# weifengliu-ssslab/Benchmark_SpMV_using_CSR5

Measured on AMD Instinct MI355X. Metric: fp64 SpMV GFLOPS, higher is better.
Workload: dtype f64

## Files before the change

### benchmark_spmv_using_csr5_amd/csrc/csr5_internal.h

```cpp
#pragma once

#include <hip/hip_runtime.h>
#include <stdint.h>

#include "csr5hip.h"

namespace csr5 {

constexpr int OMEGA = CSR5HIP_OMEGA;
#ifndef CSR5_WAVES_PER_BLOCK
#define CSR5_WAVES_PER_BLOCK 1
#endif
constexpr int WAVES_PER_BLOCK = CSR5_WAVES_PER_BLOCK;
constexpr int BLOCK = OMEGA * WAVES_PER_BLOCK;
constexpr int FMT_WAVES_PER_BLOCK = 2;
constexpr int FMT_BLOCK = OMEGA * FMT_WAVES_PER_BLOCK;
constexpr int BIT_SS = 6;
constexpr uint32_t ROW_MASK = 0x7FFFFFFFu;
constexpr int STAMP_WORD = 8;
constexpr int COUNTER_WORDS = 16;
constexpr int NUM_XCD = 8;
constexpr int RUN_SERIAL_MAX = 64;
#ifndef CSR5_XWIN_BYTES
#define CSR5_XWIN_BYTES 4096
#endif
constexpr int XWIN_BYTES = CSR5_XWIN_BYTES;
constexpr int xwin_elems(int value_size) { return XWIN_BYTES / value_size; }
constexpr int XWIN_MIN_COVER_PCT = 30;

constexpr int bit_y_of(int sigma)
{
    int base = 2, b = 1;
    while (base < OMEGA * sigma) { base *= 2; b++; }
    return b;
}
constexpr int num_packet_of(int sigma) { return (bit_y_of(sigma) + BIT_SS + sigma + 31) / 32; }

struct Geometry {
    int m, n, nnz;
    int sigma;
    int bit_y, bit_all, num_packet;
    int p;
    int tile_elems;
    int tail_start;
    int defer;
};

struct DeviceArrays {
    const int32_t *row_ptr;
    int32_t *col;
    void *val;
    uint32_t *tile_ptr;
    uint32_t *tile_desc;
    int32_t *offset_ptr;
    int32_t *offset;
    void *calibrator;
    void *carry_acc;
    uint32_t *carry_cnt;
    uint32_t *carry_meta;
    uint32_t *tile_hdr;
    uint32_t *counters;
    const int32_t *hot_cols;
    const int32_t *hot_count;
    const int32_t *hot_tile0;
    int hot_slabs, hot_capacity;
    void *range_lead;
    uint32_t *range_head;
    const uint16_t *col_lo;
    const uint8_t *col_hi;
    const int32_t *slab_off;
    int slab_shift, slab_bits;
    const void *xperm;
    const int32_t *cold_base;
    const int32_t *cold_cols;
    int cold_total;
    const float *val32;
    const uint32_t *col16;
    const int32_t *base16;
    const uint32_t *col31;
};

hipError_t launch_row_scan(const Geometry &g, const DeviceArrays &d, hipStream_t s);
hipError_t launch_tile_desc(const Geometry &g, const DeviceArrays &d, hipStream_t s);
size_t offset_scan_tmp_bytes(int entries);
hipError_t launch_offset_scan(const Geometry &g, const DeviceArrays &d, void *tmp, size_t tmp_bytes, hipStream_t s);
hipError_t launch_desc_offset(const Geometry &g, const DeviceArrays &d, hipStream_t s);
hipError_t launch_transpose(const Geometry &g, const DeviceArrays &d, int value_type, bool r2c,
                            hipStream_t s);
hipError_t launch_transpose_values(const Geometry &g, const DeviceArrays &d, int value_type, hipStream_t s);
hipError_t launch_tile_tables(const Geometry &g, const DeviceArrays &d, int value_size, uint32_t *host_words, bool export_only,
                              hipStream_t s);
hipError_t launch_col16(const Geometry &g, const DeviceArrays &d, uint32_t *col16, int32_t *base16, uint32_t *wide_tiles,
                        hipStream_t s);
constexpr int COL16_SPAN = 32768;
constexpr bool col16_sigma(int sigma) { return sigma == 8 || sigma == 12 || sigma == 16 || sigma == 24 || sigma == 32; }
hipError_t launch_col31(const Geometry &g, const DeviceArrays &d, uint32_t *col31, hipStream_t s);
constexpr bool col31_sigma(int sigma) { return sigma >= 4 && sigma <= 8; }
hipError_t launch_warmup(hipStream_t s);
hipError_t launch_validate_csr(int m, int n, int nnz, const int32_t *row_ptr, const int32_t *col, uint32_t *flag,
                               hipStream_t s);

hipError_t slab_scan_tmp_bytes(size_t items, size_t *bytes);
hipError_t slab_select_tmp_bytes(int nnz, size_t *bytes);
hipError_t slab_partition(const Geometry &g, const DeviceArrays &d, int value_type, int S, int bits, int shift,
                          uint32_t *hist, void *scan_tmp, size_t scan_tmp_bytes, int32_t *col2, void *val2,
                          uint32_t *key2, hipStream_t s);
hipError_t slab_count_segments(int nnz, const uint32_t *key2, void *tmp, unsigned int *d_count, hipStream_t s);
hipError_t slab_segments(int nnz, const uint32_t *key2, const void *tmp, int32_t *row_ptr2, unsigned char *rowidx, hipStream_t s);
size_t slab_base_words(int m, int S);
hipError_t slab_tables(int m, int m2, int nnz, int S, int p, const int32_t *row_ptr, int32_t *row_ptr2, const uint32_t *key2,
                       const uint32_t *chunk_start, uint32_t *base, uint32_t *nonempty, hipStream_t s);
hipError_t slab_hot_select(int n, int nnz, int S, int bits, int shift, int capacity, int min_count, int sample_stride,
                           const int32_t *col, uint32_t *cnt, void *hotmap, uint32_t *chist, uint32_t *thr,
                           int32_t *hot_cols, int32_t *hot_count, unsigned long long *covered, hipStream_t s);
hipError_t slab_hot_finish(int S, int p_hist, int p, int T, int nnz, int capacity, const uint32_t *chunk_start,
                           int32_t *hot_count, int32_t *tile0, int32_t *slab_off, hipStream_t s);
size_t slab_cold_words(int n, int S, int bits, int shift);
hipError_t slab_cold_sort_tmp_bytes(size_t total, int slab_bits, size_t *bytes);
hipError_t slab_hot_pack(int n, int nnz, int T, int p, int S, int bits, int shift, const int32_t *slab_off, const void *hotmap,
                         const uint32_t *cnt, const uint32_t *key2, int32_t *col2, uint16_t *col_lo, uint8_t *col_hi, uint8_t *ref, uint32_t *rank_of,
                         uint32_t *keys, uint32_t *keys_sorted, uint32_t *src_sorted, void *sort_tmp, size_t sort_tmp_bytes,
                         int32_t *cold_base, int32_t *cold_cols, hipStream_t s);
size_t slab_local_columns(int n, int bits, int shift);
size_t slab_hotmap_bytes(int n, int S, int bits, int shift);
int slab_hot_buckets();
hipError_t launch_slab_combine(int m, int tail_start, int zero_empty, int S, int value_type, const uint32_t *base,
                               const unsigned char *rowidx, const uint32_t *nonempty, const void *P, int segments, void *y,
                               hipStream_t s);

hipError_t launch_refresh_values(const Geometry &g, const uint32_t *tile_ptr, int value_type, bool pieces, const uint32_t *src,
                                 const void *in, void *out, hipStream_t s);
hipError_t refresh_map_tmp_bytes(int nnz, int bits, size_t *bytes);
hipError_t refresh_build_map(const Geometry &g, const DeviceArrays &d, int bits, int shift, void *tmp, size_t tmp_bytes,
                             uint32_t *src, hipStream_t s);

hipError_t companion_tmp_bytes(int n, int nnz, size_t *bytes);
hipError_t companion_build(const Geometry &g, const DeviceArrays &d, int value_size, void *tmp, size_t tmp_bytes,
                           int32_t *row_ptr_t, int32_t *col_t, void *val_t, uint32_t *map, hipStream_t s);
hipError_t companion_gather(int nnz, int value_size, const uint32_t *map, const void *in, void *out, hipStream_t s);

struct SpmvOptions {
    int mode;
    int xcd_remap;
    int x_window;
    int lds_y;
    int stream_nt;
    int long_runs;
    int hot;
    int col16;
    int col31;
};
constexpr int DEFER_AUTO_LONG_ROW = 128;
constexpr int DEFER_AUTO_MIN_TILES_LONG = 3000;
constexpr int DEFER_AUTO_MIN_TILE_SIGMA = 500000;
constexpr int HOT_AUTO_MIN_COVER_PCT = 25;
constexpr long long HOT_AUTO_MIN_COVERED_BEYOND = 5000000;
constexpr int HOT_LDS_BYTES = 128 * 1024;
constexpr int HOT_WAVE_LDS = 4096;
#ifndef CSR5_HOT_WAVES
#define CSR5_HOT_WAVES 8
#endif
constexpr int HOT_WAVES = CSR5_HOT_WAVES;
constexpr int HOT_WGS_PER_XCD = 32;
constexpr int HOT_RANGES_PER_SLAB = HOT_WGS_PER_XCD * HOT_WAVES;
#ifndef CSR5_HOT_DEPTH
#define CSR5_HOT_DEPTH 2
#endif
struct HotParams {
    int slabs, rounds, capacity;
    const int32_t *count;
    const int32_t *tile0;
    const uint16_t *col_lo;
    const uint8_t *col_hi;
    const int32_t *slab_off;
    const void *xp;
    const int32_t *cold_base;
    int cold_total;
};
constexpr int hot_child_sigma(int value_size) { return HOT_WAVE_LDS / (OMEGA * value_size); }
hipError_t launch_spmv(const Geometry &g, const DeviceArrays &d, int value_type, const void *x,
                       void *y, const SpmvOptions &opt, hipStream_t s);
hipError_t launch_spmm(const Geometry &g, const DeviceArrays &d, int value_type, const void *X, int ldx, int k, void *Y, int ldy,
                       void *work, int zero_empty, int xcd_remap, hipStream_t s);
constexpr int spmm_block_width(int k) { return k <= 1 ? 1 : k <= 2 ? 2 : k <= 4 ? 4 : 8; }
hipError_t launch_sddmm(const Geometry &g, const DeviceArrays &d, int value_type, const void *U, int ldu, const void *V, int ldv, int k,
                        void *out, hipStream_t s);
hipError_t launch_row_softmax(int m, const int32_t *row_ptr, int value_type, const void *scores, void *out, hipStream_t s);
hipError_t launch_row_softmax_grad(int m, const int32_t *row_ptr, int value_type, const void *p, const void *g, void *out,
                                   hipStream_t s);
struct AttCall {
    int heads, groups, k, d;
    const void *Q;
    int ldq;
    const void *K;
    int ldk;
    const void *V;
    int ldv;
    void *O;
    int ldo;
    double scale;
    const void *slopes;
    const void *B;
    int ldb;
    const void *a;
    double negative_slope;
};
struct AttBwdCall : AttCall {
    const void *dO;
    int lddo;
    void *dQ;
    int lddq;
    void *dK;
    int lddk;
    void *dV;
    int lddv;
    void *work;
    void *dS;
    int ldds;
    void *dAr;
    int lddar;
    const Geometry *gt;
    const DeviceArrays *dt;
    const uint32_t *map;
};
enum AttVariant { ATT_PLAIN, ATT_BIASED, ATT_EDGE, ATT_GAT };
using AttLaunch = hipError_t(const Geometry &, const DeviceArrays &, const AttCall &, hipStream_t);
using AttBwdLaunch = hipError_t(const Geometry &, const DeviceArrays &, const AttBwdCall &, hipStream_t);
hipError_t launch_mha(const Geometry &g, const DeviceArrays &d, int value_type, const AttCall &c, hipStream_t s);
hipError_t launch_mha_biased(const Geometry &g, const DeviceArrays &d, int value_type, const AttCall &c, hipStream_t s);
hipError_t launch_mha_edge(const Geometry &g, const DeviceArrays &d, int value_type, const AttCall &c, hipStream_t s);
hipError_t launch_gat(const Geometry &g, const DeviceArrays &d, int value_type, const AttCall &c, hipStream_t s);
hipError_t launch_mha_lowp(const Geometry &g, const DeviceArrays &d, int operand_type, const AttCall &c, hipStream_t s);
hipError_t launch_mha_bwd(const Geometry &g, const DeviceArrays &d, int value_type, const AttBwdCall &c, hipStream_t s);
hipError_t launch_mha_biased_bwd(const Geometry &g, const DeviceArrays &d, int value_type, const AttBwdCall &c, hipStream_t s);
hipError_t launch_mha_edge_bwd(const Geometry &g, const DeviceArrays &d, int value_type, const AttBwdCall &c, hipStream_t s);
hipError_t launch_gat_bwd(const Geometry &g, const DeviceArrays &d, int value_type, const AttBwdCall &c, hipStream_t s);
hipError_t launch_mha_lowp_bwd(const Geometry &g, const DeviceArrays &d, int operand_type, const AttBwdCall &c, hipStream_t s);
hipError_t launch_spmv_hot(const Geometry &g, const DeviceArrays &d, int value_type, const void *x, void *y,
                           const SpmvOptions &opt, hipStream_t s);
hipError_t prepare_spmv_hot(const Geometry &g, const DeviceArrays &d, int value_type, const SpmvOptions &opt);
hipError_t launch_fp32_exact(const double *v, size_t n, unsigned *flag, hipStream_t s);
hipError_t launch_narrow(const double *v, size_t n, float *o, int tile_elems, int transposed_tiles, hipStream_t s);
hipError_t launch_range_heads(const Geometry &g, const DeviceArrays &d, hipStream_t s);
hipError_t launch_x_permute(const Geometry &g, const DeviceArrays &d, int value_type, const void *x, hipStream_t s);

}
```

### benchmark_spmv_using_csr5_amd/csrc/csr5_slab.hip

```cpp
#include "csr5_internal.h"
#include "csr5_slabmap.h"

#include <rocprim/device/device_radix_sort.hpp>
#include <rocprim/device/device_scan.hpp>
#include <rocprim/iterator/counting_iterator.hpp>

namespace csr5 {

constexpr int SLAB_BLOCK = 256;
constexpr int SLAB_MAX = 64;
constexpr uint32_t SLAB_KEY_FIRST = 0x80000000u;

__host__ __device__ inline size_t slab_hot_groups(int n, int shift, int bits) { return (slab_local_count(n, shift, bits) + 127) / 128; }
__device__ __forceinline__ bool hot_lookup(const uint4 w, uint32_t bit, uint32_t &below)
{
    const unsigned long long lo = (unsigned long long)w.x | ((unsigned long long)w.y << 32);
    const unsigned long long hi = (unsigned long long)w.z | ((unsigned long long)w.w << 32);
    const unsigned long long word = bit < 64 ? lo : hi;
    const uint32_t b = bit & 63;
    below = (uint32_t)__popcll(word & ((1ull << b) - 1ull)) + (bit < 64 ? 0u : (uint32_t)__popcll(lo));
    return (word >> b) & 1ull;
}

__device__ __forceinline__ int upper_bound_i32(const int32_t *__restrict__ a, int key, int size)
{
    int lo = 0, hi = size;
    while (lo < hi) {
        const int mid = (int)(((unsigned)lo + (unsigned)hi) >> 1);
        if (a[mid] <= key)
            lo = mid + 1;
        else
            hi = mid;
    }
    return lo;
}

__device__ __forceinline__ bool tile_is_transposed(const Geometry &g, const uint32_t *tile_ptr, int t)
{
    return t < g.p - 1 && tile_ptr[t] != tile_ptr[t + 1];
}

constexpr int HIST_TILES = 16, HIST_PAD = OMEGA + 1;
__global__ void __launch_bounds__(SLAB_BLOCK)
k_slab_hist(Geometry g, const int32_t *__restrict__ col, int S, int bits, int shift, uint32_t *__restrict__ hist)
{
    extern __shared__ uint32_t hist_lds[];
    __shared__ uint32_t sh[SLAB_MAX][HIST_TILES];
    const int lane = threadIdx.x & (OMEGA - 1), wave = threadIdx.x >> 6;
    uint32_t *mine = hist_lds + (size_t)wave * S * HIST_PAD;
    const int t0 = blockIdx.x * HIST_TILES;
    for (int i = wave; i < HIST_TILES; i += SLAB_BLOCK / OMEGA) {
        const int t = t0 + i;
        uint32_t total = 0;
        if (t < g.p) {
            for (int k = 0; k < S; k++)
                mine[k * HIST_PAD + lane] = 0;
            const size_t base = (size_t)t * g.tile_elems;
            const int E = (int)((size_t)g.nnz - base < (size_t)g.tile_elems ? (size_t)g.nnz - base : (size_t)g.tile_elems);
            constexpr int AHEAD = 8;
            for (int q0 = 0; q0 < E; q0 += AHEAD * OMEGA) {
                int32_t c[AHEAD];
#pragma unroll
                for (int u = 0; u < AHEAD; u++) {
                    const int q = q0 + u * OMEGA + lane;
                    c[u] = col[base + (q < E ? q : E - 1)];
                }
#pragma unroll
                for (int u = 0; u < AHEAD; u++)
                    if (q0 + u * OMEGA + lane < E)
                        atomicAdd(&mine[slab_of((uint32_t)c[u], shift, bits) * HIST_PAD + lane], 1u);
            }
            if (lane < S)
                for (int j = 0; j < OMEGA; j++)
                    total += mine[lane * HIST_PAD + j];
        }
        if (lane < S)
            sh[lane][i] = total;
    }
    __syncthreads();
    for (int e = threadIdx.x; e < S * HIST_TILES; e += SLAB_BLOCK) {
        const int k = e / HIST_TILES, i = e % HIST_TILES;
        if (t0 + i < g.p)
            hist[(size_t)k * g.p + t0 + i] = sh[k][i];
    }
}

__device__ __forceinline__ unsigned long long same_slab_lanes(int k, bool valid, int bits)
{
    unsigned long long same = __ballot(valid);
    for (int b = 0; b < bits; b++) {
        const bool on = (k >> b) & 1;
        const unsigned long long bal = __ballot(on);
        same &= on ? bal : ~bal;
    }
    return same;
}

template <typename VT>
__global__ void __launch_bounds__(SLAB_BLOCK)
k_slab_scatter(Geometry g, const int32_t *__restrict__ row_ptr, const uint32_t *__restrict__ tile_ptr,
               const int32_t *__restrict__ col, const VT *__restrict__ val, int S, int bits, int shift,
               const uint32_t *__restrict__ chunk_start, int32_t *__restrict__ col2, VT *__restrict__ val2,
               uint32_t *__restrict__ key2)
{
    extern __shared__ __attribute__((aligned(16))) char smem[];
    const int T = g.tile_elems;
    VT *sval = reinterpret_cast<VT *>(smem);
    int32_t *scol = reinterpret_cast<int32_t *>(smem + (size_t)T * sizeof(VT));
    uint32_t *off = reinterpret_cast<uint32_t *>(smem + (size_t)T * (sizeof(VT) + 4));
    uint16_t *inv = reinterpret_cast<uint16_t *>(off + (size_t)(T / OMEGA) * S);
    unsigned char *skey = reinterpret_cast<unsigned char *>(inv + T);
    unsigned char *srank = skey + T;
    constexpr int ROWCAP = 1024;
    __shared__ int32_t srow[ROWCAP];
    __shared__ uint32_t slab_first[SLAB_MAX], gstart[SLAB_MAX], lstart[SLAB_MAX + 1];

    const int t = blockIdx.x;
    const int tid = threadIdx.x, lane = tid & (OMEGA - 1), wave = tid >> 6;
    const size_t base = (size_t)t * T;
    const int E = (int)((size_t)g.nnz - base < (size_t)T ? (size_t)g.nnz - base : (size_t)T);
    const bool tr = tile_is_transposed(g, tile_ptr, t);
    for (int q = tid; q < E; q += SLAB_BLOCK) {
        const int c = tr ? (q & (OMEGA - 1)) * g.sigma + (q >> 6) : q;
        const int32_t ci = col[base + q];
        scol[c] = ci;
        sval[c] = val[base + q];
        skey[c] = (unsigned char)slab_of((uint32_t)ci, shift, bits);
    }
    if (tid < S) {
        slab_first[tid] = chunk_start[(size_t)tid * g.p];
        gstart[tid] = chunk_start[(size_t)tid * g.p + t];
    }
    const int rs = (int)(tile_ptr[t] & ROW_MASK);
    const int re = (int)(tile_ptr[t + 1] & ROW_MASK);
    const bool rows_in_lds = re - rs <= ROWCAP;
    if (rows_in_lds)
        for (int i = tid; i < re - rs; i += SLAB_BLOCK)
            srow[i] = row_ptr[rs + 1 + i];
    __syncthreads();
    const int nchunks = (E + OMEGA - 1) / OMEGA;
    for (int ch = wave; ch < nchunks; ch += SLAB_BLOCK / OMEGA) {
        const int c = ch * OMEGA + lane;
        const bool valid = c < E;
        const int k = valid ? skey[c] : 0;
        if (lane < S)
            off[ch * S + lane] = 0;
        const unsigned long long same = same_slab_lanes(k, valid, bits);
        if (valid) {
            const int rank = __popcll(same & ((1ull << lane) - 1ull));
            srank[c] = (unsigned char)rank;
            if (rank == 0)
                off[ch * S + k] = (uint32_t)__popcll(same);
        }
    }
    __syncthreads();
    if (tid < S) {
        uint32_t run = 0;
        for (int ch = 0; ch < nchunks; ch++) {
            const uint32_t v = off[ch * S + tid];
            off[ch * S + tid] = run;
            run += v;
        }
        lstart[tid + 1] = run;
    }
    __syncthreads();
    if (tid == 0) {
        lstart[0] = 0;
        for (int k = 0; k < S; k++)
            lstart[k + 1] += lstart[k];
    }
    __syncthreads();
    for (int c = tid; c < E; c += SLAB_BLOCK) {
        const int k = skey[c];
        inv[lstart[k] + off[(c >> 6) * S + k] + srank[c]] = (uint16_t)c;
    }
    __syncthreads();
    for (int o = tid; o < E; o += SLAB_BLOCK) {
        const int c = inv[o];
        const int k = skey[c];
        const size_t dst = (size_t)gstart[k] + ((uint32_t)o - lstart[k]);
        const int j = (int)(base + c);
        const int row = rs + (rows_in_lds ? upper_bound_i32(srow, j, re - rs) : upper_bound_i32(row_ptr + rs + 1, j, re - rs));
        col2[dst] = scol[c];
        val2[dst] = sval[c];
        key2[dst] = (uint32_t)row | (dst == slab_first[k] ? SLAB_KEY_FIRST : 0u);
    }
}

__device__ __forceinline__ bool key_starts(uint32_t a, uint32_t before)
{
    return (a & SLAB_KEY_FIRST) != 0 || ((a ^ before) & ~SLAB_KEY_FIRST) != 0;
}
__device__ __forceinline__ unsigned segment_starts4(const uint32_t *__restrict__ key, long long j, long long hi, uint32_t k[4])
{
    if (j >= hi)
        return 0u;
    const uint32_t before = j > 0 ? key[j - 1] : 0u;
    if (j + 4 <= hi) {
        const uint4 v = *reinterpret_cast<const uint4 *>(key + j);
        k[0] = v.x, k[1] = v.y, k[2] = v.z, k[3] = v.w;
    } else {
        for (int i = 0; i < 4; i++)
            k[i] = j + i < hi ? key[j + i] : 0u;
    }
    unsigned f = j == 0 || key_starts(k[0], before) ? 1u : 0u;
#pragma unroll
    for (int i = 1; i < 4; i++)
        f |= (j + i < hi && key_starts(k[i], k[i - 1]) ? 1u : 0u) << i;
    return f;
}

constexpr int COMBINE_ROWS = 256;

constexpr int SEG_BLOCKS = 2048;
constexpr int SEG_STEP = SLAB_BLOCK * 4;
__host__ __device__ inline long long seg_chunk(int nnz, int blocks)
{
    long long c = ((long long)nnz + blocks - 1) / blocks;
    return (c + SEG_STEP - 1) / SEG_STEP * SEG_STEP;
}
static int seg_blocks(int nnz)
{
    long long b = ((long long)nnz + 4095) / 4096;
    return (int)(b < 1 ? 1 : (b > SEG_BLOCKS ? SEG_BLOCKS : b));
}

__global__ void __launch_bounds__(SLAB_BLOCK)
k_slab_count_segments(int nnz, const uint32_t *__restrict__ key, unsigned int *__restrict__ block_count)
{
    __shared__ unsigned part[SLAB_BLOCK / OMEGA];
    const long long chunk = seg_chunk(nnz, gridDim.x);
    const long long lo = (long long)blockIdx.x * chunk, hi = lo + chunk < nnz ? lo + chunk : nnz;
    unsigned local = 0;
    for (long long j = lo + (long long)threadIdx.x * 4; j < hi; j += SEG_STEP) {
        uint32_t k[4];
        local += (unsigned)__popc(segment_starts4(key, j, hi, k));
    }
#pragma unroll
    for (int d = 32; d >= 1; d >>= 1)
        local += __shfl_xor(local, d, OMEGA);
    if ((threadIdx.x & (OMEGA - 1)) == 0)
        part[threadIdx.x / OMEGA] = local;
    __syncthreads();
    if (threadIdx.x == 0) {
        unsigned total = 0;
        for (int w = 0; w < SLAB_BLOCK / OMEGA; w++)
            total += part[w];
        block_count[blockIdx.x] = total;
    }
}

__global__ void __launch_bounds__(1024) k_slab_scan_counts(int blocks, unsigned int *__restrict__ block_count,
                                                           unsigned int *__restrict__ total)
{
    __shared__ unsigned wave_total[16];
    const int per = (blocks + 1023) / 1024;
    const int first = (int)threadIdx.x * per;
    unsigned v[2] = {0u, 0u};
    for (int i = 0; i < per; i++)
        if (first + i < blocks)
            v[i] = block_count[first + i];
    const unsigned sum = v[0] + v[1];
    const int lane = threadIdx.x & (OMEGA - 1), w = threadIdx.x >> 6;
    unsigned incl = sum;
#pragma unroll
    for (int d = 1; d < OMEGA; d <<= 1) {
        const unsigned o = __shfl_up(incl, d, OMEGA);
        if (lane >= d)
            incl += o;
    }
    if (lane == OMEGA - 1)
        wave_total[w] = incl;
    __syncthreads();
    unsigned run = incl - sum;
    for (int k = 0; k < w; k++)
        run += wave_total[k];
    for (int i = 0; i < per; i++)
        if (first + i < blocks) {
            block_count[first + i] = run;
            run += v[i];
        }
    if (threadIdx.x == 1023) {
        block_count[blocks] = run;
        *total = run;
    }
}

__global__ void __launch_bounds__(SLAB_BLOCK)
k_slab_emit_segments(int nnz, const uint32_t *__restrict__ key, const unsigned int *__restrict__ block_offset,
                     int32_t *__restrict__ row_ptr2, unsigned char *__restrict__ rowidx)
{
    __shared__ unsigned wave_count[SLAB_BLOCK / OMEGA];
    const long long chunk = seg_chunk(nnz, gridDim.x);
    const long long lo = (long long)blockIdx.x * chunk, hi = lo + chunk < nnz ? lo + chunk : nnz;
    const int lane = threadIdx.x & (OMEGA - 1), w = threadIdx.x / OMEGA;
    unsigned out = block_offset[blockIdx.x];
    for (long long j0 = lo; j0 < hi; j0 += SEG_STEP) {
        const long long j = j0 + (long long)threadIdx.x * 4;
        uint32_t k4[4];
        const unsigned f = segment_starts4(key, j, hi, k4);
        const unsigned own = (unsigned)__popc(f);
        unsigned incl = own;
#pragma unroll
        for (int d = 1; d < OMEGA; d <<= 1) {
            const unsigned o = __shfl_up(incl, d, OMEGA);
            if (lane >= d)
                incl += o;
        }
        if (lane == OMEGA - 1)
            wave_count[w] = incl;
        __syncthreads();
        unsigned before = 0, all = 0;
        for (int k = 0; k < SLAB_BLOCK / OMEGA; k++) {
            before += k < w ? wave_count[k] : 0u;
            all += wave_count[k];
        }
        unsigned at = out + before + incl - own;
#pragma unroll
        for (int i = 0; i < 4; i++)
            if (f & (1u << i)) {
                row_ptr2[at] = (int32_t)(j + i);
                rowidx[at++] = (unsigned char)(k4[i] & (COMBINE_ROWS - 1));
            }
        out += all;
        __syncthreads();
    }
}

__global__ void __launch_bounds__(SLAB_BLOCK)
k_slab_base(int m2, int nnz, int S, int nblk, const int32_t *__restrict__ row_ptr2, const uint32_t *__restrict__ key,
            const uint32_t *__restrict__ chunk_start, int p, uint32_t *__restrict__ base, int32_t *__restrict__ row_ptr2_end)
{
    __shared__ int slab_seg[SLAB_MAX + 1];
    if (blockIdx.x == 0 && threadIdx.x == 0)
        *row_ptr2_end = nnz;
    if ((int)threadIdx.x <= S) {
        const uint32_t first = (int)threadIdx.x < S ? chunk_start[(size_t)threadIdx.x * p] : (uint32_t)nnz;
        int lo = 0, hi = m2;
        while (lo < hi) {
            const int mid = (int)(((unsigned)lo + (unsigned)hi) >> 1);
            if ((uint32_t)row_ptr2[mid] < first)
                lo = mid + 1;
            else
                hi = mid;
        }
        slab_seg[threadIdx.x] = lo;
    }
    __syncthreads();
    const long long e = (long long)blockIdx.x * SLAB_BLOCK + threadIdx.x;
    if (e >= (long long)(nblk + 1) * S)
        return;
    const int b = (int)(e / S), k = (int)(e % S);
    const uint32_t want = (uint32_t)b * COMBINE_ROWS;
    int lo = slab_seg[k], hi = slab_seg[k + 1];
    while (lo < hi) {
        const int mid = (int)(((unsigned)lo + (unsigned)hi) >> 1);
        if ((key[row_ptr2[mid]] & ~SLAB_KEY_FIRST) < want)
            lo = mid + 1;
        else
            hi = mid;
    }
    base[e] = (uint32_t)lo;
}

__global__ void __launch_bounds__(SLAB_BLOCK)
k_slab_nonempty(int m, const int32_t *__restrict__ row_ptr, uint32_t *__restrict__ bits)
{
    const int r = blockIdx.x * SLAB_BLOCK + threadIdx.x;
    const bool on = r < m && row_ptr[r + 1] > row_ptr[r];
    const unsigned long long b = __ballot(on);
    const int lane = threadIdx.x & (OMEGA - 1);
    if ((lane & 31) == 0 && r < m + 32)
        bits[r >> 5] = (uint32_t)(b >> lane);
}

#if defined(CSR5_COMBINE_STAMPS)
__device__ unsigned long long g_combine_stamps[2 * (1 << 17)];
__device__ unsigned long long g_combine_phase[4 * (1 << 17)];
#define COMBINE_PHASE(i)                                                                                               \
    do {                                                                                                               \
        asm volatile("s_waitcnt vmcnt(0) lgkmcnt(0)" ::: "memory");                                                    \
        if (lane == 0 && blk < (1 << 17))                                                                              \
            g_combine_phase[4 * blk + (i)] = wall_clock64();                                                           \
    } while (0)
extern "C" int csr5hip_debug_combine_phase(unsigned long long *dst, int count)
{
    return (int)hipMemcpyFromSymbol(dst, HIP_SYMBOL(g_combine_phase), (size_t)count * sizeof(unsigned long long));
}
extern "C" int csr5hip_debug_combine_stamps(unsigned long long *dst, int count)
{
    return (int)hipMemcpyFromSymbol(dst, HIP_SYMBOL(g_combine_stamps), (size_t)count * sizeof(unsigned long long));
}
#else
#define COMBINE_PHASE(i)
#endif

#ifndef CSR5_COMBINE_WAVES
#define CSR5_COMBINE_WAVES 4
#endif
constexpr int COMBINE_WAVES = CSR5_COMBINE_WAVES;
template <typename VT, int S>
__device__ __forceinline__ void combine_block(int blk, int lane, VT *acc, int m, int tail_start, int zero_empty, int m2,
                                              const uint32_t *__restrict__ base, const unsigned char *__restrict__ rowidx,
                                              const uint32_t *__restrict__ nonempty, const VT *__restrict__ P,
                                              VT *__restrict__ y)
{
    const int r0 = blk * COMBINE_ROWS;
    constexpr int BW = (2 * S + OMEGA - 1) / OMEGA;
    uint32_t bw[BW];
#pragma unroll
    for (int i = 0; i < BW; i++) {
        const int e = i * OMEGA + lane;
        bw[i] = base[(size_t)blk * S + (e < 2 * S ? e : 0)];
    }
    uint32_t ne[COMBINE_ROWS / OMEGA];
#pragma unroll
    for (int j = 0; j < COMBINE_ROWS / OMEGA; j++)
        ne[j] = nonempty[(r0 >> 5) + 2 * j + (lane >> 5)];
#pragma unroll
    for (int j = 0; j < COMBINE_ROWS / OMEGA; j++)
        acc[j * OMEGA + lane] = 0;
    COMBINE_PHASE(0);
    auto bound = [&](int e) -> int { return __builtin_amdgcn_readlane((int)bw[e / OMEGA], e % OMEGA); };
    constexpr int G = S < 16 ? S : 16;
    const unsigned dummy = COMBINE_ROWS + lane;
#pragma unroll
    for (int k0 = 0; k0 < S; k0 += G) {
        int lo[G], len[G], longest = 0;
#pragma unroll
        for (int q = 0; q < G; q++) {
            lo[q] = bound(k0 + q);
            len[q] = bound(S + k0 + q) - lo[q];
            longest = len[q] > longest ? len[q] : longest;
        }
        for (int off = 0; off < longest; off += OMEGA) {
            VT part[G];
            unsigned idx[G];
#pragma unroll
            for (int q = 0; q < G; q++) {
                int j = off + lane < len[q] ? off + lane : len[q] - 1;
                j += lo[q];
                j = j < 0 ? 0 : (j < m2 ? j : m2 - 1);
                part[q] = P[j];
                idx[q] = rowidx[j];
            }
            COMBINE_PHASE(1);
#pragma unroll
            for (int q = 0; q < G; q++) {
                const unsigned slot = off + lane < len[q] ? idx[q] : dummy;
                acc[slot] += part[q];
            }
        }
    }
    COMBINE_PHASE(2);
    __builtin_amdgcn_fence(__ATOMIC_RELEASE, "wavefront");
    __builtin_amdgcn_wave_barrier();
#pragma unroll
    for (int j = 0; j < COMBINE_ROWS / OMEGA; j++) {
        const int r = r0 + j * OMEGA + lane;
        if (r < m) {
            if ((ne[j] >> (lane & 31)) & 1u)
                y[r] = acc[j * OMEGA + lane];
            else if (zero_empty || r >= tail_start)
                y[r] = 0;
        }
    }
}

template <typename VT, int S>
__global__ void __launch_bounds__(COMBINE_WAVES * OMEGA)
k_slab_combine(int m, int tail_start, int zero_empty, int m2, const uint32_t *__restrict__ base,
               const unsigned char *__restrict__ rowidx, const uint32_t *__restrict__ nonempty,
               const VT *__restrict__ P, VT *__restrict__ y)
{
    __shared__ VT acc_all[COMBINE_WAVES][COMBINE_ROWS + OMEGA];
    const int lane = threadIdx.x & (OMEGA - 1), w = threadIdx.x >> 6;
    int wg = blockIdx.x;
    {
        const int octet = wg >> 3;
        if ((octet << 3) + 8 <= (int)gridDim.x)
            wg = (octet << 3) + (((wg & 7) + (int)(((unsigned)octet * 0x9E3779B1u) >> 29)) & 7);
    }
    const int blk = wg * COMBINE_WAVES + w;
    const int r0 = blk * COMBINE_ROWS;
    if (r0 >= m)
        return;
#if defined(CSR5_COMBINE_STAMPS)
    if (lane == 0 && blk < (1 << 17))
        g_combine_stamps[2 * blk] = wall_clock64();
#endif
    combine_block<VT, S>(blk, lane, acc_all[w], m, tail_start, zero_empty, m2, base, rowidx, nonempty, P, y);
#if defined(CSR5_COMBINE_STAMPS)
    if (lane == 0 && blk < (1 << 17))
        g_combine_stamps[2 * blk + 1] = wall_clock64();
#endif
}


template <typename VT, int S>
__global__ void __launch_bounds__(COMBINE_WAVES * OMEGA)
k_slab_combine_persistent(int m, int tail_start, int zero_empty, int m2, const uint32_t *__restrict__ base,
                          const unsigned char *__restrict__ rowidx, const uint32_t *__restrict__ nonempty,
                          const VT *__restrict__ P, VT *__restrict__ y, unsigned *__restrict__ ticket)
{
    __shared__ VT acc_all[COMBINE_WAVES][COMBINE_ROWS + OMEGA];
    const int lane = threadIdx.x & (OMEGA - 1), w = threadIdx.x >> 6;
    const unsigned nblk = (unsigned)((m + COMBINE_ROWS - 1) / COMBINE_ROWS), nwaves = gridDim.x * COMBINE_WAVES;
#if defined(CSR5_COMBINE_STATIC)
    const unsigned g = blockIdx.x * COMBINE_WAVES + w;
    for (unsigned k = 0; k * nwaves < nblk; k++) {
        const unsigned t = k * nwaves + (g + (k * 0x9E3779B1u >> 8)) % nwaves;
        if (t < nblk) {
            combine_block<VT, S>((int)t, lane, acc_all[w], m, tail_start, zero_empty, m2, base, rowidx, nonempty, P, y);
            __builtin_amdgcn_fence(__ATOMIC_ACQUIRE, "wavefront");
            __builtin_amdgcn_wave_barrier();
        }
    }
    (void)ticket;
    return;
#endif
    auto draw = [&]() -> unsigned {
        unsigned t = 0;
        if (lane == 0)
            t = __hip_atomic_fetch_add(ticket, 1u, __ATOMIC_RELAXED, __HIP_MEMORY_SCOPE_AGENT);
        return (unsigned)__builtin_amdgcn_readfirstlane((int)t);
    };
    unsigned t = draw();
    while (t < nblk) {
        const unsigned next = draw();
        combine_block<VT, S>((int)t, lane, acc_all[w], m, tail_start, zero_empty, m2, base, rowidx, nonempty, P, y);
        __builtin_amdgcn_fence(__ATOMIC_ACQUIRE, "wavefront");
        __builtin_amdgcn_wave_barrier();
        t = next;
    }
    if (t == nblk + nwaves - 1u && lane == 0)
        __hip_atomic_store(ticket, 0u, __ATOMIC_RELAXED, __HIP_MEMORY_SCOPE_AGENT);
}

constexpr int HOT_BUCKETS = 2048;

constexpr int COUNT_SLOTS = 16384, COUNT_BLOCK = 1024, COUNT_WGS = 256, COUNT_AHEAD = 4;
__global__ void __launch_bounds__(COUNT_BLOCK)
k_col_count(int nnz, int stride, const int32_t *__restrict__ col, uint32_t *__restrict__ cnt)
{
    extern __shared__ uint32_t count_lds[];
    uint32_t *key = count_lds, *hits = count_lds + COUNT_SLOTS;
    for (int i = threadIdx.x; i < COUNT_SLOTS; i += COUNT_BLOCK) {
        key[i] = 0xFFFFFFFFu;
        hits[i] = 0;
    }
    __syncthreads();
    const size_t chunks = ((size_t)nnz + OMEGA - 1) / OMEGA;
    const size_t sampled = (chunks + stride - 1) / stride;
    const int lane = threadIdx.x & (OMEGA - 1);
    const size_t step = (size_t)gridDim.x * (COUNT_BLOCK / OMEGA);
    for (size_t w0 = ((size_t)blockIdx.x * COUNT_BLOCK + threadIdx.x) / OMEGA; w0 < sampled; w0 += step * COUNT_AHEAD) {
        uint32_t c[COUNT_AHEAD];
#pragma unroll
        for (int u = 0; u < COUNT_AHEAD; u++) {
            const size_t w = w0 + u * step;
            const size_t i = w * stride * OMEGA + lane;
            c[u] = w < sampled && i < (size_t)nnz ? (uint32_t)col[i] : 0xFFFFFFFFu;
        }
#pragma unroll
        for (int u = 0; u < COUNT_AHEAD; u++) {
            if (c[u] == 0xFFFFFFFFu)
                continue;
            const uint32_t slot = (c[u] * 2654435761u) >> 18;
            const uint32_t owner = atomicCAS(&key[slot], 0xFFFFFFFFu, c[u]);
            if (owner == 0xFFFFFFFFu || owner == c[u])
                atomicAdd(&hits[slot], 1u);
            else
                atomicAdd(&cnt[c[u]], 1u);
        }
    }
    __syncthreads();
    for (int i = threadIdx.x; i < COUNT_SLOTS; i += COUNT_BLOCK)
        if (hits[i])
            atomicAdd(&cnt[key[i]], hits[i]);
}

constexpr int HOT_LOW = 64;
constexpr int HOT_HIST_COLS = 4096;
__global__ void __launch_bounds__(SLAB_BLOCK)
k_hot_hist(int n, const uint32_t *__restrict__ cnt, int S, int bits, int shift, uint32_t *__restrict__ chist)
{
    __shared__ uint32_t low[SLAB_MAX * HOT_LOW];
    for (int i = threadIdx.x; i < S * HOT_LOW; i += SLAB_BLOCK)
        low[i] = 0;
    __syncthreads();
    const int first = blockIdx.x * HOT_HIST_COLS;
    for (int c = first + threadIdx.x; c < first + HOT_HIST_COLS && c < n; c += SLAB_BLOCK) {
        const uint32_t v = cnt[c];
        if (!v)
            continue;
        const uint32_t k = slab_of((uint32_t)c, shift, bits);
        if (v < HOT_LOW)
            atomicAdd(&low[k * HOT_LOW + v], 1u);
        else
            atomicAdd(&chist[(size_t)k * HOT_BUCKETS + (v < HOT_BUCKETS - 1 ? v : HOT_BUCKETS - 1)], 1u);
    }
    __syncthreads();
    for (int i = threadIdx.x; i < S * HOT_LOW; i += SLAB_BLOCK)
        if (low[i])
            atomicAdd(&chist[(size_t)(i / HOT_LOW) * HOT_BUCKETS + i % HOT_LOW], low[i]);
}

__global__ void __launch_bounds__(OMEGA)
k_hot_threshold(int capacity, int min_count, const uint32_t *__restrict__ chist, uint32_t *__restrict__ thr)
{
    constexpr int PER = HOT_BUCKETS / OMEGA;
    const int lane = threadIdx.x;
    const uint32_t *h = chist + (size_t)blockIdx.x * HOT_BUCKETS + lane * PER;
    uint32_t v[PER];
    unsigned long long own = 0;
#pragma unroll
    for (int i = 0; i < PER; i++) {
        v[i] = h[i];
        own += v[i];
    }
    unsigned long long incl = own;
#pragma unroll
    for (int d = 1; d < OMEGA; d <<= 1) {
        const unsigned long long o = __shfl_down(incl, d, OMEGA);
        if (lane + d < OMEGA)
            incl += o;
    }
    unsigned long long total = incl - own;
    int best = HOT_BUCKETS;
#pragma unroll
    for (int i = PER - 1; i >= 0; i--) {
        total += v[i];
        const int b = lane * PER + i;
        if (b >= min_count && total <= (unsigned long long)(capacity - 1))
            best = b;
    }
#pragma unroll
    for (int d = 32; d >= 1; d >>= 1) {
        const int o = __shfl_xor(best, d, OMEGA);
        best = o < best ? o : best;
    }
    unsigned long long at_best = 0;
    {
        unsigned long long run = incl - own;
#pragma unroll
        for (int i = PER - 1; i >= 0; i--) {
            run += v[i];
            if (lane * PER + i == best)
                at_best = run;
        }
    }
#pragma unroll
    for (int d = 32; d >= 1; d >>= 1)
        at_best += __shfl_xor(at_best, d, OMEGA);
    if (lane == 0) {
        thr[blockIdx.x] = (uint32_t)best;
        thr[gridDim.x + blockIdx.x] = (uint32_t)((unsigned long long)(capacity - 1) - at_best);
    }
}

constexpr int HOT_ASSIGN_COLS = 16384;
__global__ void __launch_bounds__(SLAB_BLOCK)
k_hot_assign(int n, int S, const uint32_t *__restrict__ cnt, int bits, int shift, const uint32_t *__restrict__ thr,
             int min_count, int32_t *__restrict__ fill, uint32_t *__restrict__ hotbits, size_t G,
             unsigned long long *__restrict__ covered)
{
    __shared__ int want[SLAB_MAX], base[SLAB_MAX], given[SLAB_MAX];
    if (threadIdx.x < SLAB_MAX)
        want[threadIdx.x] = given[threadIdx.x] = base[threadIdx.x] = 0;
    __syncthreads();
    const int first = blockIdx.x * HOT_ASSIGN_COLS;
    const int last = first + HOT_ASSIGN_COLS < n ? first + HOT_ASSIGN_COLS : n;
    auto chosen = [&](int c, uint32_t &k, uint32_t &v) -> int {
        v = cnt[c];
        if (!v)
            return 0;
        k = slab_of((uint32_t)c, shift, bits);
        const uint32_t bucket = v < HOT_BUCKETS - 1 ? v : HOT_BUCKETS - 1;
        const uint32_t b = thr[k];
        return bucket >= b ? 1 : (bucket + 1 == b && (int)bucket >= min_count ? 2 : 0);
    };
    auto mark = [&](int c, uint32_t k) {
        const uint32_t local = slab_local((uint32_t)c, shift, bits);
        atomicOr(&hotbits[(size_t)k * G * 4 + (local >> 5)], 1u << (local & 31));
    };
    uint32_t k = 0, v = 0;
    unsigned long long got = 0;
    for (int c = first + (int)threadIdx.x; c < last; c += SLAB_BLOCK) {
        const int cls = chosen(c, k, v);
        if (cls == 1) {
            mark(c, k);
            got += v;
        } else if (cls == 2) {
            atomicAdd(&want[k], 1);
        }
    }
    __syncthreads();
    if (threadIdx.x < SLAB_MAX && want[threadIdx.x])
        base[threadIdx.x] = atomicAdd(&fill[threadIdx.x], want[threadIdx.x]);
    __syncthreads();
    for (int c = first + (int)threadIdx.x; c < last; c += SLAB_BLOCK)
        if (chosen(c, k, v) == 2 && want[k] && base[k] + atomicAdd(&given[k], 1) < (int)thr[S + k]) {
            mark(c, k);
            got += v;
        }
#pragma unroll
    for (int d = 32; d >= 1; d >>= 1)
        got += __shfl_xor(got, d, OMEGA);
    if ((threadIdx.x & (OMEGA - 1)) == 0 && got)
        atomicAdd(covered, got);
}

__global__ void __launch_bounds__(SLAB_MAX + 1)
k_hot_finish(int S, int p_hist, int p, int T, int nnz, int capacity, const uint32_t *__restrict__ chunk_start,
             int32_t *__restrict__ hot_count, int32_t *__restrict__ tile0, int32_t *__restrict__ slab_off)
{
    const int k = threadIdx.x;
    if (k > S)
        return;
    const long long off = k < S ? (long long)chunk_start[(size_t)k * p_hist] : (long long)nnz;
    slab_off[k] = (int32_t)off;
    long long t = (off + T - 1) / T;
    tile0[k] = (int32_t)(t < p - 1 ? t : p - 1);
    if (k < S && hot_count[k] > capacity)
        hot_count[k] = capacity;
}

constexpr int RANK_BLOCK = 1024;
__global__ void __launch_bounds__(RANK_BLOCK)
k_hot_rank(int bits, int shift, int capacity, size_t G, const uint4 *__restrict__ hotbits, uint16_t *__restrict__ pre,
           int32_t *__restrict__ hot_cols, int32_t *__restrict__ hot_count)
{
    __shared__ uint32_t wave_total[RANK_BLOCK / OMEGA];
    const uint32_t k = blockIdx.x;
    const size_t g0 = (size_t)blockIdx.y * RANK_BLOCK;
    const int lane = threadIdx.x & (OMEGA - 1), w = threadIdx.x / OMEGA;
    auto bits_of = [](const uint4 v) { return (uint32_t)(__popc(v.x) + __popc(v.y) + __popc(v.z) + __popc(v.w)); };
    auto block_scan = [&](uint32_t own, uint32_t &before, uint32_t &all) {
        uint32_t incl = own;
#pragma unroll
        for (int d = 1; d < OMEGA; d <<= 1) {
            const uint32_t o = __shfl_up(incl, d, OMEGA);
            if (lane >= d)
                incl += o;
        }
        __syncthreads();
        if (lane == OMEGA - 1)
            wave_total[w] = incl;
        __syncthreads();
        before = incl - own;
        all = 0;
        for (int i = 0; i < RANK_BLOCK / OMEGA; i++) {
            before += i < w ? wave_total[i] : 0u;
            all += wave_total[i];
        }
    };
    uint32_t front = 0;
    for (size_t g = threadIdx.x; g < g0; g += RANK_BLOCK)
        front += bits_of(hotbits[(size_t)k * G + g]);
    uint32_t unused, running;
    block_scan(front, unused, running);
    running += 1;
    const size_t g = g0 + threadIdx.x;
    uint4 v = make_uint4(0, 0, 0, 0);
    if (g < G)
        v = hotbits[(size_t)k * G + g];
    uint32_t before, all;
    block_scan(bits_of(v), before, all);
    uint32_t slot = running + before;
    if (g < G) {
        pre[(size_t)k * G + g] = (uint16_t)slot;
        const uint32_t word[4] = {v.x, v.y, v.z, v.w};
#pragma unroll
        for (int i = 0; i < 4; i++) {
            uint32_t m = word[i];
            while (m) {
                const uint32_t b = (uint32_t)__builtin_ctz(m);
                m &= m - 1;
                if ((int)slot < capacity)
                    hot_cols[(size_t)k * capacity + slot] = (int32_t)slab_column(k, (uint32_t)g * 128u + i * 32u + b, shift, bits);
                slot++;
            }
        }
    }
    if (blockIdx.y == gridDim.y - 1 && threadIdx.x == 0)
        hot_count[k] = (int32_t)(running + all);
}

constexpr int ENCODE_BLOCK = 1024, ENCODE_WGS_PER_XCD = 32, ENCODE_UNROLL = 4;
constexpr int ENC_MARK = 1, ENC_PACK = 2;
template <bool IN_LDS, int MODE>
__global__ void __launch_bounds__(ENCODE_BLOCK)
k_hot_encode(int nnz, int T, int p, int S, int bits, int shift, const int32_t *__restrict__ slab_off,
             const uint4 *__restrict__ hotbits, const uint16_t *__restrict__ hotpre, size_t G, int32_t *__restrict__ col2,
             uint16_t *__restrict__ col_lo, uint8_t *__restrict__ col_hi, uint8_t *__restrict__ ref,
             const uint32_t *__restrict__ rank_of, size_t L, const uint32_t *__restrict__ key)
{
    extern __shared__ __attribute__((aligned(16))) char smem[];
    uint4 *lbits = reinterpret_cast<uint4 *>(smem);
    uint16_t *lpre = reinterpret_cast<uint16_t *>(smem + G * sizeof(uint4));
    __shared__ int32_t soff[SLAB_MAX + 1];
    if ((int)threadIdx.x <= S)
        soff[threadIdx.x] = slab_off[threadIdx.x];
    __syncthreads();
    const int xcd = blockIdx.x % NUM_XCD, j = blockIdx.x / NUM_XCD, nj = gridDim.x / NUM_XCD;
    const long long last = (long long)(p - 1) * T;
    for (int mine = xcd; mine < S; mine += NUM_XCD) {
        const uint4 *gb = hotbits + (size_t)mine * G;
        const uint16_t *gp = hotpre + (size_t)mine * G;
        if (IN_LDS) {
            __syncthreads();
            for (size_t g = threadIdx.x; g < G; g += ENCODE_BLOCK) {
                lbits[g] = gb[g];
                if (MODE != ENC_MARK)
                    lpre[g] = gp[g];
            }
            __syncthreads();
        }
        const long long own_end = soff[mine + 1];
        auto slot_of = [&](uint32_t local) -> int {
            const uint32_t g = local >> 7;
            uint32_t below;
            const bool hot = hot_lookup(IN_LDS ? lbits[g] : gb[g], local & 127u, below);
            if (MODE == ENC_MARK)
                return hot ? 0 : -1;
            return hot ? (int)((uint32_t)(IN_LDS ? lpre[g] : gp[g]) + below) : -1;
        };
        auto encode = [&](int32_t c, long long pos) -> int32_t {
            const uint32_t local = slab_local((uint32_t)c, shift, bits);
            const int slot = pos < own_end ? slot_of(local) : -1;
            if (slot >= 0)
                return (int32_t)(0x800000u | (uint32_t)slot);
            const size_t at = (size_t)(pos < own_end ? (uint32_t)mine : slab_of((uint32_t)c, shift, bits)) * L + local;
            if (MODE == ENC_MARK) {
                ref[at] = 1;
                return 0;
            }
            return (int32_t)rank_of[at];
        };
        const long long begin = ((long long)soff[mine] + T - 1) / T * T;
        long long end = (own_end + T - 1) / T * T;
        end = end < last ? end : last;
        if (begin >= end)
            continue;
        int4 *c4 = reinterpret_cast<int4 *>(col2 + begin);
        uint2 *lo4 = reinterpret_cast<uint2 *>(col_lo + begin);
        uint32_t *hi4 = reinterpret_cast<uint32_t *>(col_hi + begin);
        const long long quads = (end - begin) / 4;
        for (long long q0 = (long long)j * ENCODE_BLOCK * ENCODE_UNROLL; q0 < quads;
             q0 += (long long)nj * ENCODE_BLOCK * ENCODE_UNROLL) {
            int4 v[ENCODE_UNROLL];
#pragma unroll
            for (int u = 0; u < ENCODE_UNROLL; u++) {
                const long long q = q0 + u * ENCODE_BLOCK + threadIdx.x;
                if (q < quads)
                    v[u] = c4[q];
            }
#pragma unroll
            for (int u = 0; u < ENCODE_UNROLL; u++) {
                const long long q = q0 + u * ENCODE_BLOCK + threadIdx.x;
                if (q < quads) {
                    const long long pos = begin + q * 4;
                    v[u].x = encode(v[u].x, pos);
                    v[u].y = encode(v[u].y, pos + 1);
                    v[u].z = encode(v[u].z, pos + 2);
                    v[u].w = encode(v[u].w, pos + 3);
                    if (MODE == ENC_PACK) {
                        uint32_t k4[4];
                        const unsigned st = segment_starts4(key, pos, (long long)nnz, k4);
                        const uint32_t a = (uint32_t)v[u].x | ((st & 1u) << 22), b = (uint32_t)v[u].y | (((st >> 1) & 1u) << 22),
                                       c = (uint32_t)v[u].z | (((st >> 2) & 1u) << 22), d = (uint32_t)v[u].w | (((st >> 3) & 1u) << 22);
                        lo4[q] = make_uint2((a & 0xFFFFu) | (b << 16), (c & 0xFFFFu) | (d << 16));
                        hi4[q] = ((a >> 16) & 0xFFu) | (((b >> 16) & 0xFFu) << 8) | (((c >> 16) & 0xFFu) << 16) | ((d >> 16) << 24);
                    }
                }
            }
        }
    }
}

constexpr uint32_t COLD_COUNT_CAP = 1023, COLD_KEY_BITS = 11;
__global__ void __launch_bounds__(SLAB_BLOCK)
k_cold_keys(size_t total, size_t L, int n, int bits, int shift, const uint8_t *__restrict__ ref, const uint32_t *__restrict__ cnt,
            uint32_t *__restrict__ keys)
{
    const size_t i = (size_t)blockIdx.x * SLAB_BLOCK + threadIdx.x;
    if (i >= total)
        return;
    const uint32_t k = (uint32_t)(i / L);
    uint32_t low = COLD_COUNT_CAP + 1;
    if (ref[i]) {
        const uint32_t col = slab_column(k, (uint32_t)(i - (size_t)k * L), shift, bits);
        const uint32_t c = col < (uint32_t)n ? cnt[col] : 0u;
        low = COLD_COUNT_CAP - (c < COLD_COUNT_CAP ? c : COLD_COUNT_CAP);
    }
    keys[i] = (k << COLD_KEY_BITS) | low;
}
__global__ void __launch_bounds__(SLAB_MAX)
k_cold_layout(int S, size_t L, const uint32_t *__restrict__ keys_sorted, int32_t *__restrict__ cold_base)
{
    __shared__ int32_t n[SLAB_MAX];
    const int k = threadIdx.x;
    if (k < S) {
        const uint32_t none = ((uint32_t)k << COLD_KEY_BITS) | (COLD_COUNT_CAP + 1);
        size_t lo = (size_t)k * L, hi = lo + L;
        while (lo < hi) {
            const size_t mid = (lo + hi) >> 1;
            if (keys_sorted[mid] < none)
                lo = mid + 1;
            else
                hi = mid;
        }
        n[k] = (int32_t)(lo - (size_t)k * L);
    }
    __syncthreads();
    if (k == 0) {
        int32_t run = 0;
        for (int i = 0; i < S; i++) {
            cold_base[i] = run;
            run += n[i];
        }
        cold_base[S] = run;
    }
}
__global__ void __launch_bounds__(SLAB_BLOCK)
k_cold_rank(size_t total, size_t L, int bits, int shift, const uint32_t *__restrict__ src_sorted,
            const int32_t *__restrict__ cold_base, uint32_t *__restrict__ rank_of, int32_t *__restrict__ cold_cols)
{
    const size_t q = (size_t)blockIdx.x * SLAB_BLOCK + threadIdx.x;
    if (q >= total)
        return;
    const uint32_t k = (uint32_t)(q / L);
    const uint32_t r = (uint32_t)(q - (size_t)k * L);
    const int32_t b = cold_base[k];
    if ((int32_t)r >= cold_base[k + 1] - b)
        return;
    const uint32_t src = src_sorted[q];
    rank_of[src] = r;
    cold_cols[(size_t)b + r] = (int32_t)slab_column(k, (uint32_t)(src - (size_t)k * L), shift, bits);
}

size_t slab_scatter_lds(const Geometry &g, int S, size_t vsize)
{
    const size_t T = (size_t)g.tile_elems;
    return T * (vsize + 4) + (T / OMEGA) * (size_t)S * 4 + T * 2 + T + T;
}

hipError_t slab_partition(const Geometry &g, const DeviceArrays &d, int value_type, int S, int bits, int shift,
                          uint32_t *hist, void *scan_tmp, size_t scan_tmp_bytes, int32_t *col2, void *val2,
                          uint32_t *key2, hipStream_t s)
{
    const size_t hist_lds = (size_t)(SLAB_BLOCK / OMEGA) * S * HIST_PAD * 4;
    hipError_t e = hipFuncSetAttribute(reinterpret_cast<const void *>(k_slab_hist), hipFuncAttributeMaxDynamicSharedMemorySize,
                                       (int)hist_lds);
    if (e != hipSuccess)
        return e;
    hipLaunchKernelGGL(k_slab_hist, dim3((g.p + HIST_TILES - 1) / HIST_TILES), dim3(SLAB_BLOCK), hist_lds, s, g, d.col, S, bits, shift,
                       hist);
    e = hipGetLastError();
    if (e != hipSuccess)
        return e;
    e = rocprim::exclusive_scan(scan_tmp, scan_tmp_bytes, hist, hist, 0u, (size_t)S * g.p, rocprim::plus<uint32_t>(), s);
    if (e != hipSuccess)
        return e;
    const size_t vs = value_type == CSR5HIP_F64 ? 8 : 4;
    const size_t lds = slab_scatter_lds(g, S, vs);
    if (value_type == CSR5HIP_F64)
        hipLaunchKernelGGL(k_slab_scatter<double>, dim3(g.p), dim3(SLAB_BLOCK), lds, s, g, d.row_ptr, d.tile_ptr, d.col,
                           (const double *)d.val, S, bits, shift, hist, col2, (double *)val2, key2);
    else
        hipLaunchKernelGGL(k_slab_scatter<float>, dim3(g.p), dim3(SLAB_BLOCK), lds, s, g, d.row_ptr, d.tile_ptr, d.col,
                           (const float *)d.val, S, bits, shift, hist, col2, (float *)val2, key2);
    return hipGetLastError();
}

hipError_t slab_scan_tmp_bytes(size_t items, size_t *bytes)
{
    uint32_t *null_u = nullptr;
    return rocprim::exclusive_scan(nullptr, *bytes, null_u, null_u, 0u, items, rocprim::plus<uint32_t>(), nullptr);
}

hipError_t slab_select_tmp_bytes(int nnz, size_t *bytes)
{
    *bytes = ((size_t)seg_blocks(nnz) + 1) * 4;
    return hipSuccess;
}

hipError_t slab_count_segments(int nnz, const uint32_t *key2, void *tmp, unsigned int *d_count, hipStream_t s)
{
    const int blocks = seg_blocks(nnz);
    hipLaunchKernelGGL(k_slab_count_segments, dim3(blocks), dim3(SLAB_BLOCK), 0, s, nnz, key2, (unsigned int *)tmp);
    hipLaunchKernelGGL(k_slab_scan_counts, dim3(1), dim3(1024), 0, s, blocks, (unsigned int *)tmp, d_count);
    return hipGetLastError();
}

hipError_t slab_segments(int nnz, const uint32_t *key2, const void *tmp, int32_t *row_ptr2, unsigned char *rowidx, hipStream_t s)
{
    hipLaunchKernelGGL(k_slab_emit_segments, dim3(seg_blocks(nnz)), dim3(SLAB_BLOCK), 0, s, nnz, key2,
                       (const unsigned int *)tmp, row_ptr2, rowidx);
    return hipGetLastError();
}

size_t slab_base_words(int m, int S) { return ((size_t)(m + COMBINE_ROWS - 1) / COMBINE_ROWS + 2) * (size_t)S; }
hipError_t slab_tables(int m, int m2, int nnz, int S, int p, const int32_t *row_ptr, int32_t *row_ptr2, const uint32_t *key2,
                       const uint32_t *chunk_start, uint32_t *base, uint32_t *nonempty, hipStream_t s)
{
    const int nblk = (m + COMBINE_ROWS - 1) / COMBINE_ROWS;
    const long long entries = (long long)(nblk + 1) * S;
    hipLaunchKernelGGL(k_slab_base, dim3((unsigned)((entries + SLAB_BLOCK - 1) / SLAB_BLOCK)), dim3(SLAB_BLOCK), 0, s, m2, nnz, S,
                       nblk, row_ptr2, key2, chunk_start, p, base, row_ptr2 + m2);
    hipLaunchKernelGGL(k_slab_nonempty, dim3((m + 32 + SLAB_BLOCK - 1) / SLAB_BLOCK), dim3(SLAB_BLOCK), 0, s, m, row_ptr, nonempty);
    return hipGetLastError();
}

#if defined(CSR5_COMBINE_PERSISTENT)
__device__ unsigned g_combine_ticket = 0;
#endif
template <typename VT>
static hipError_t combine_typed(int m, int tail_start, int zero_empty, int S, int m2, const uint32_t *base,
                                const unsigned char *rowidx, const uint32_t *nonempty, const void *P, void *y, hipStream_t s)
{
    const int rows_per_block = COMBINE_ROWS * COMBINE_WAVES;
    const dim3 grid((m + rows_per_block - 1) / rows_per_block), block(COMBINE_WAVES * OMEGA);
#if defined(CSR5_COMBINE_PERSISTENT)
    if (S == 16 && (int)grid.x > CSR5_COMBINE_PERSISTENT * 256) {
        unsigned *ticket = nullptr;
        hipError_t e = hipGetSymbolAddress((void **)&ticket, HIP_SYMBOL(g_combine_ticket));
        if (e != hipSuccess)
            return e;
        hipLaunchKernelGGL((k_slab_combine_persistent<VT, 16>), dim3(CSR5_COMBINE_PERSISTENT * 256), block, 0, s, m, tail_start,
                           zero_empty, m2, base, rowidx, nonempty, (const VT *)P, (VT *)y, ticket);
        return hipGetLastError();
    }
#endif
    switch (S) {
#define CSR5_SLAB_CASE(N)                                                                                              \
    case N:                                                                                                            \
        hipLaunchKernelGGL((k_slab_combine<VT, N>), grid, block, 0, s, m, tail_start, zero_empty, m2, base, rowidx,    \
                           nonempty, (const VT *)P, (VT *)y);                                                          \
        break;
        CSR5_SLAB_CASE(2) CSR5_SLAB_CASE(4) CSR5_SLAB_CASE(8) CSR5_SLAB_CASE(16) CSR5_SLAB_CASE(32) CSR5_SLAB_CASE(64)
#undef CSR5_SLAB_CASE
    default: return hipErrorInvalidValue;
    }
    return hipGetLastError();
}

hipError_t launch_slab_combine(int m, int tail_start, int zero_empty, int S, int value_type, const uint32_t *base,
                               const unsigned char *rowidx, const uint32_t *nonempty, const void *P, int segments, void *y,
                               hipStream_t s)
{
    if (m <= 0 || segments <= 0)
        return hipSuccess;
    return value_type == CSR5HIP_F64 ? combine_typed<double>(m, tail_start, zero_empty, S, segments, base, rowidx, nonempty, P, y, s)
                                     : combine_typed<float>(m, tail_start, zero_empty, S, segments, base, rowidx, nonempty, P, y, s);
}

}

namespace csr5 {

hipError_t slab_hot_select(int n, int nnz, int S, int bits, int shift, int capacity, int min_count, int sample_stride,
                           const int32_t *col, uint32_t *cnt, void *hotmap, uint32_t *chist, uint32_t *thr,
                           int32_t *hot_cols, int32_t *hot_count, unsigned long long *covered, hipStream_t s)
{
    const size_t G = slab_hot_groups(n, shift, bits);
    uint4 *hotbits = (uint4 *)hotmap;
    uint16_t *hotpre = (uint16_t *)(hotbits + (size_t)S * G);
    long long blocks = ((long long)nnz / sample_stride + COUNT_BLOCK * 8 - 1) / (COUNT_BLOCK * 8);
    blocks = blocks < 1 ? 1 : (blocks > COUNT_WGS ? COUNT_WGS : blocks);
    const size_t count_lds = (size_t)COUNT_SLOTS * 8;
    hipError_t ea = hipFuncSetAttribute(reinterpret_cast<const void *>(k_col_count), hipFuncAttributeMaxDynamicSharedMemorySize,
                                        (int)count_lds);
    if (ea != hipSuccess)
        return ea;
    hipError_t e = hipMemsetAsync(hot_count, 0, (size_t)S * 4, s);
    if (e != hipSuccess)
        return e;
    hipLaunchKernelGGL(k_col_count, dim3((unsigned)blocks), dim3(COUNT_BLOCK), count_lds, s, nnz, sample_stride, col, cnt);
    hipLaunchKernelGGL(k_hot_hist, dim3((n + HOT_HIST_COLS - 1) / HOT_HIST_COLS), dim3(SLAB_BLOCK), 0, s, n, cnt, S, bits, shift,
                       chist);
    hipLaunchKernelGGL(k_hot_threshold, dim3(S), dim3(OMEGA), 0, s, capacity, min_count, chist, thr);
    hipLaunchKernelGGL(k_hot_assign, dim3((n + HOT_ASSIGN_COLS - 1) / HOT_ASSIGN_COLS), dim3(SLAB_BLOCK), 0, s, n, S, cnt, bits, shift,
                       thr, min_count, hot_count, (uint32_t *)hotbits, G, covered);
    hipLaunchKernelGGL(k_hot_rank, dim3(S, (unsigned)((G + RANK_BLOCK - 1) / RANK_BLOCK)), dim3(RANK_BLOCK), 0, s, bits, shift,
                       capacity, G, hotbits, hotpre, hot_cols, hot_count);
    return hipGetLastError();
}

hipError_t slab_hot_finish(int S, int p_hist, int p, int T, int nnz, int capacity, const uint32_t *chunk_start,
                           int32_t *hot_count, int32_t *tile0, int32_t *slab_off, hipStream_t s)
{
    hipLaunchKernelGGL(k_hot_finish, dim3(1), dim3(SLAB_MAX + 1), 0, s, S, p_hist, p, T, nnz, capacity, chunk_start,
                       hot_count, tile0, slab_off);
    return hipGetLastError();
}

static hipError_t hot_encode_pass(int mode, int n, int nnz, int T, int p, int S, int bits, int shift, const int32_t *slab_off,
                                  const void *hotmap, int32_t *col2, uint16_t *col_lo, uint8_t *col_hi, uint8_t *ref,
                                  const uint32_t *rank_of, const uint32_t *key, hipStream_t s)
{
    const size_t G = slab_hot_groups(n, shift, bits);
    const size_t L = slab_local_count(n, shift, bits);
    const uint4 *hotbits = (const uint4 *)hotmap;
    const uint16_t *hotpre = (const uint16_t *)(hotbits + (size_t)S * G);
    const size_t lds = G * (sizeof(uint4) + sizeof(uint16_t));
    const dim3 grid(NUM_XCD * ENCODE_WGS_PER_XCD), block(ENCODE_BLOCK);
    const bool in_lds = lds <= 150 * 1024;
    auto launch = [&](auto kern) -> hipError_t {
        if (in_lds) {
            hipError_t e = hipFuncSetAttribute(reinterpret_cast<const void *>(kern), hipFuncAttributeMaxDynamicSharedMemorySize,
                                               (int)lds);
            if (e != hipSuccess)
                return e;
        }
        hipLaunchKernelGGL(kern, grid, block, in_lds ? lds : 0, s, nnz, T, p, S, bits, shift, slab_off, hotbits, hotpre, G, col2,
                           col_lo, col_hi, ref, rank_of, L, key);
        return hipGetLastError();
    };
    if (mode == ENC_MARK)
        return in_lds ? launch(k_hot_encode<true, ENC_MARK>) : launch(k_hot_encode<false, ENC_MARK>);
    return in_lds ? launch(k_hot_encode<true, ENC_PACK>) : launch(k_hot_encode<false, ENC_PACK>);
}

size_t slab_cold_words(int n, int S, int bits, int shift) { return (size_t)S * slab_local_count(n, shift, bits); }
hipError_t slab_cold_sort_tmp_bytes(size_t total, int slab_bits, size_t *bytes)
{
    uint32_t *nu = nullptr;
    rocprim::counting_iterator<uint32_t> iota(0u);
    return rocprim::radix_sort_pairs(nullptr, *bytes, nu, nu, iota, nu, total, 0, slab_bits + (int)COLD_KEY_BITS, nullptr);
}

hipError_t slab_hot_pack(int n, int nnz, int T, int p, int S, int bits, int shift, const int32_t *slab_off, const void *hotmap,
                         const uint32_t *cnt, const uint32_t *key2, int32_t *col2, uint16_t *col_lo, uint8_t *col_hi, uint8_t *ref, uint32_t *rank_of,
                         uint32_t *keys, uint32_t *keys_sorted, uint32_t *src_sorted, void *sort_tmp, size_t sort_tmp_bytes,
                         int32_t *cold_base, int32_t *cold_cols, hipStream_t s)
{
    const size_t L = slab_local_count(n, shift, bits), total = (size_t)S * L;
    hipError_t e = hot_encode_pass(ENC_MARK, n, nnz, T, p, S, bits, shift, slab_off, hotmap, col2, nullptr, nullptr, ref, nullptr, nullptr, s);
    if (e != hipSuccess)
        return e;
    const unsigned blocks = (unsigned)((total + SLAB_BLOCK - 1) / SLAB_BLOCK);
    hipLaunchKernelGGL(k_cold_keys, dim3(blocks), dim3(SLAB_BLOCK), 0, s, total, L, n, bits, shift, ref, cnt, keys);
    rocprim::counting_iterator<uint32_t> iota(0u);
    e = rocprim::radix_sort_pairs(sort_tmp, sort_tmp_bytes, keys, keys_sorted, iota, src_sorted, total, 0, bits + (int)COLD_KEY_BITS, s);
    if (e != hipSuccess)
        return e;
    hipLaunchKernelGGL(k_cold_layout, dim3(1), dim3(SLAB_MAX), 0, s, S, L, keys_sorted, cold_base);
    hipLaunchKernelGGL(k_cold_rank, dim3(blocks), dim3(SLAB_BLOCK), 0, s, total, L, bits, shift, src_sorted, cold_base, rank_of, cold_cols);
    e = hipGetLastError();
    if (e != hipSuccess)
        return e;
    return hot_encode_pass(ENC_PACK, n, nnz, T, p, S, bits, shift, slab_off, hotmap, col2, col_lo, col_hi, nullptr, rank_of, key2, s);
}

size_t slab_local_columns(int n, int bits, int shift) { return slab_local_count(n, shift, bits); }

size_t slab_hotmap_bytes(int n, int S, int bits, int shift)
{
    return (size_t)S * slab_hot_groups(n, shift, bits) * (sizeof(uint4) + sizeof(uint16_t)) + 256;
}

int slab_hot_buckets() { return HOT_BUCKETS; }

}
```

### benchmark_spmv_using_csr5_amd/csrc/csr5_slab_build.hip

```cpp
#include <algorithm>
#include <string>
#include <vector>

#include "csr5_handle.h"

using namespace csr5;

static_assert(PLAN_OMEGA == OMEGA && PLAN_NUM_XCD == NUM_XCD && PLAN_HOT_LDS_BYTES == HOT_LDS_BYTES && PLAN_HOT_WAVE_LDS == HOT_WAVE_LDS &&
                  PLAN_HOT_WAVES == HOT_WAVES && PLAN_HOT_RANGES_PER_SLAB == HOT_RANGES_PER_SLAB &&
                  PLAN_HOT_AUTO_MIN_COVER_PCT == HOT_AUTO_MIN_COVER_PCT && PLAN_HOT_AUTO_MIN_COVERED_BEYOND == HOT_AUTO_MIN_COVERED_BEYOND &&
                  plan_hot_child_sigma(8) == hot_child_sigma(8) && plan_hot_child_sigma(4) == hot_child_sigma(4),
              "csr5_slab_plan.h restates constants of csr5_internal.h: keep them equal");

namespace csr5 {

void SlabStructure::release()
{
    if (child) {
        csr5hip_free(child);
        child = nullptr;
    }
    values_narrowed = false;
    refresh_map_valid = false;
    for (Buffer &b : buf)
        b.release();
    S = 0;
    m2 = 0;
    hot_cover_pct = 0;
}

void SlabStructure::deactivate()
{
    if (child) {
        child->drop_graphs();
        child->format = -1;
        child->hot_enabled = false;
    }
    S = 0;
    m2 = 0;
    hot_cover_pct = 0;
    refresh_map_valid = false;
}

long long SlabStructure::bytes() const
{
    long long sum = child ? (long long)child->b_arena.cap : 0;
    for (const Buffer &b : buf)
        sum += (long long)b.cap;
    return sum;
}

}

namespace {

struct SlabBuild {
    csr5hip_handle h;
    SlabPlan plan;
    SlabTmpSizes sz;
    SlabArena arena;
    size_t tmp_keep;
    SlabChoice choice;
    unsigned int m2;
    void *tmp(SlabRegion r) const { return (char *)h->slab[B_TMP].ptr + arena.off[r]; }
    void *covered() const { return (char *)h->slab[B_TMP].ptr + arena.covered(); }
};

int plan_slabs(csr5hip_handle h, SlabPlan *plan)
{
    SlabInputs in{};
    in.m = h->g.m, in.n = h->g.n, in.nnz = h->g.nnz, in.p = h->g.p, in.sigma = h->g.sigma, in.tile_elems = h->g.tile_elems;
    in.value_size = (int)h->vsize();
    in.xwin_covered = h->xwin_covered;
    in.req = h->req;
    in.mode = h->opt.mode;
    in.is_child = h->is_child;
    const int S = slab_count_for(in);
    if (S && slab_table_possible(in, S)) {
        int dev = 0;
        HIP_TRY(hipGetDevice(&dev));
        HIP_TRY(hipDeviceGetAttribute(&in.lds_max, hipDeviceAttributeMaxSharedMemoryPerBlock, dev));
    }
    *plan = slab_plan(in);
    return CSR5HIP_SUCCESS;
}

int reserve_temporaries(SlabBuild &b)
{
    csr5hip_handle h = b.h;
    const Geometry &g = h->g;
    const SlabPlan &pl = b.plan;
    if (!h->device_total_bytes) {
        size_t free_b = 0, total_b = 0;
        (void)hipMemGetInfo(&free_b, &total_b);
        h->device_total_bytes = total_b ? total_b : 1;
    }
    b.tmp_keep = std::max((size_t)64 << 20, h->device_total_bytes / 64);
    SlabTmpSizes &sz = b.sz;
    HIP_TRY(slab_scan_tmp_bytes((size_t)pl.S_alloc * g.p, &sz.scan));
    HIP_TRY(slab_select_tmp_bytes(g.nnz, &sz.select));
    sz.hot_buckets = slab_hot_buckets();
    sz.hotmap = slab_hotmap_bytes(g.n, pl.S_alloc, pl.bits_alloc, h->req.slab_shift);
    if (pl.hot) {
        sz.cold_words = slab_cold_words(g.n, pl.S, pl.bits_s, h->req.slab_shift);
        HIP_TRY(slab_cold_sort_tmp_bytes(sz.cold_words, pl.bits_s, &sz.cold_sort));
    }
    sz.base_words = slab_base_words(g.m, pl.S_alloc);
    b.arena = slab_arena(pl, sz);
    if (h->req.slab_mem_mib > 0 && !slab_memory_fits(slab_memory_need(pl, sz, b.arena.total), h->req.slab_mem_mib))
        return fail_hip(hipErrorOutOfMemory, "column slabs: CSR5HIP_OPT_SLAB_MEMORY_MIB");
    HIP_TRY(h->slab[B_TMP].reserve(b.arena.total));
    return CSR5HIP_SUCCESS;
}

int select_hot_columns(SlabBuild &b)
{
    csr5hip_handle h = b.h;
    SlabStructure &sl = h->slab;
    const Geometry &g = h->g;
    const SlabPlan &pl = b.plan;
    hipStream_t s = h->stream;
    const int S = pl.S, shift = h->req.slab_shift;
    HIP_TRY(sl[B_HOT_COLS].reserve((size_t)S * pl.hot_capacity * 4));
    HIP_TRY(sl[B_HOT_COUNT].reserve((size_t)S * 4));
    HIP_TRY(sl[B_HOT_TILE0].reserve(((size_t)2 * S + 1) * 4));
    HIP_TRY(sl[B_SLAB_OFF].reserve(((size_t)S + 1) * 4));
    HIP_TRY(sl[B_LEAD].reserve((size_t)S * HOT_RANGES_PER_SLAB * h->vsize()));
    HIP_TRY(sl[B_RANGE_HEAD].reserve(((size_t)S * HOT_RANGES_PER_SLAB + 1) * 4));
    HIP_TRY(hipMemsetAsync(b.tmp(T_CNT), 0, b.arena.bytes[T_CNT], s));
    HIP_TRY(hipMemsetAsync(b.tmp(T_HOTMAP), 0, slab_hotmap_bytes(g.n, S, pl.bits_s, shift), s));
    HIP_TRY(hipMemsetAsync(b.tmp(T_CHIST), 0, (size_t)S * slab_hot_buckets() * 4, s));
    HIP_TRY(hipMemsetAsync(b.covered(), 0, 8, s));
    HIP_TRY(hipMemsetAsync(sl[B_HOT_COLS].ptr, 0, (size_t)S * pl.hot_capacity * 4, s));
    HIP_TRY(slab_hot_select(g.n, g.nnz, S, pl.bits_s, shift, pl.hot_capacity, pl.min_count, pl.stride, (const int32_t *)h->d.col,
                            (uint32_t *)b.tmp(T_CNT), b.tmp(T_HOTMAP), (uint32_t *)b.tmp(T_CHIST), (uint32_t *)b.tmp(T_THR),
                            (int32_t *)sl[B_HOT_COLS].ptr, (int32_t *)sl[B_HOT_COUNT].ptr, (unsigned long long *)b.covered(), s));
    unsigned long long covered = 0;
    HIP_TRY(hipMemcpyAsync(&covered, b.covered(), 8, hipMemcpyDeviceToHost, s));
    HIP_TRY(hipStreamSynchronize(s));
    sl.hot_cover_pct = slab_cover_pct(pl, covered);
    return CSR5HIP_SUCCESS;
}

int partition_segments(SlabBuild &b)
{
    csr5hip_handle h = b.h;
    SlabStructure &sl = h->slab;
    const Geometry &g = h->g;
    hipStream_t s = h->stream;
    const int S = b.choice.S;
    const uint32_t *key = (const uint32_t *)b.tmp(T_KEY), *hist = (const uint32_t *)b.tmp(T_HIST);
    HIP_TRY(sl[B_COL2].reserve((size_t)g.nnz * 4));
    HIP_TRY(sl[B_VAL2].reserve((size_t)g.nnz * h->vsize()));
    HIP_TRY(slab_partition(g, h->d, h->value_type, S, b.choice.bits, h->req.slab_shift, (uint32_t *)b.tmp(T_HIST), b.tmp(T_SCAN), b.sz.scan,
                           (int32_t *)sl[B_COL2].ptr, sl[B_VAL2].ptr, (uint32_t *)b.tmp(T_KEY), s));
    HIP_TRY(slab_count_segments(g.nnz, key, b.tmp(T_SEL), (unsigned int *)b.tmp(T_COUNT), s));
    unsigned int m2 = 0;
    HIP_TRY(hipMemcpyAsync(&m2, b.tmp(T_COUNT), 4, hipMemcpyDeviceToHost, s));
    HIP_TRY(hipStreamSynchronize(s));
    b.m2 = m2;
    HIP_TRY(sl[B_ROW_PTR2].reserve(((size_t)m2 + 1) * 4));
    HIP_TRY(sl[B_ROWIDX].reserve((size_t)m2 + 1));
    HIP_TRY(slab_segments(g.nnz, key, b.tmp(T_SEL), (int32_t *)sl[B_ROW_PTR2].ptr, (unsigned char *)sl[B_ROWIDX].ptr, s));
    HIP_TRY(sl[B_BASE].reserve(slab_base_words(g.m, S) * 4));
    HIP_TRY(sl[B_NONEMPTY].reserve(((size_t)g.m / 32 + 16) * 4));
    HIP_TRY(slab_tables(g.m, (int)m2, g.nnz, S, g.p, h->d.row_ptr, (int32_t *)sl[B_ROW_PTR2].ptr, key, hist, (uint32_t *)sl[B_BASE].ptr,
                        (uint32_t *)sl[B_NONEMPTY].ptr, s));
    HIP_TRY(sl[B_P].reserve(((size_t)m2 + 1) * h->vsize()));
    HIP_TRY(hipMemsetAsync(sl[B_P].ptr, 0, ((size_t)m2 + 1) * h->vsize(), s));
    return CSR5HIP_SUCCESS;
}

int deal_and_pack(SlabBuild &b)
{
    csr5hip_handle h = b.h;
    SlabStructure &sl = h->slab;
    const Geometry &g = h->g;
    const SlabPlan &pl = b.plan;
    hipStream_t s = h->stream;
    const int S = b.choice.S;
    HIP_TRY(slab_hot_finish(S, g.p, pl.hot_p, pl.hot_T, g.nnz, pl.hot_capacity, (const uint32_t *)b.tmp(T_HIST), (int32_t *)sl[B_HOT_COUNT].ptr,
                            (int32_t *)sl[B_HOT_TILE0].ptr, (int32_t *)sl[B_SLAB_OFF].ptr, s));
    std::vector<int32_t> first_tile((size_t)S + 1);
    HIP_TRY(hipMemcpyAsync(first_tile.data(), sl[B_HOT_TILE0].ptr, ((size_t)S + 1) * 4, hipMemcpyDeviceToHost, s));
    HIP_TRY(hipStreamSynchronize(s));
    const std::vector<int> order = slab_deal(first_tile, S);
    HIP_TRY(hipMemcpyAsync((int32_t *)sl[B_HOT_TILE0].ptr + S + 1, order.data(), (size_t)S * 4, hipMemcpyHostToDevice, s));
    int32_t cold_total = 0;
    HIP_TRY(sl[B_COL_LO].reserve((size_t)g.nnz * 2 + 64));
    HIP_TRY(sl[B_COL_HI].reserve((size_t)g.nnz + 64));
    const size_t cold_cap = std::min(b.sz.cold_words, (size_t)g.nnz);
    HIP_TRY(sl[B_COLD_BASE].reserve(((size_t)S + 1) * 4));
    HIP_TRY(sl[B_COLD_COLS].reserve((cold_cap + 1) * 4));
    HIP_TRY(sl[B_XPERM].reserve(((size_t)S * pl.hot_capacity + cold_cap + (size_t)pl.hot_T + 1) * h->vsize()));
    HIP_TRY(hipMemsetAsync(b.tmp(T_REF), 0, b.sz.cold_words, s));
    HIP_TRY(slab_hot_pack(g.n, g.nnz, pl.hot_T, pl.hot_p, S, b.choice.bits, h->req.slab_shift, (const int32_t *)sl[B_SLAB_OFF].ptr,
                          b.tmp(T_HOTMAP), (const uint32_t *)b.tmp(T_CNT), (const uint32_t *)b.tmp(T_KEY), (int32_t *)sl[B_COL2].ptr,
                          (uint16_t *)sl[B_COL_LO].ptr, (uint8_t *)sl[B_COL_HI].ptr, (uint8_t *)b.tmp(T_REF), (uint32_t *)b.tmp(T_RANK),
                          (uint32_t *)b.tmp(T_KEYS), (uint32_t *)b.tmp(T_KEYS2), (uint32_t *)b.tmp(T_SRC), b.tmp(T_SORT), b.sz.cold_sort,
                          (int32_t *)sl[B_COLD_BASE].ptr, (int32_t *)sl[B_COLD_COLS].ptr, s));
    HIP_TRY(hipMemcpyAsync(&cold_total, (int32_t *)sl[B_COLD_BASE].ptr + S, 4, hipMemcpyDeviceToHost, s));
    HIP_TRY(hipStreamSynchronize(s));
    sl.cold_total = cold_total;
    return CSR5HIP_SUCCESS;
}

void inherit_child(csr5hip_handle c, const csr5hip_handle_s *h)
{
    c->req = Requests{};
    c->req.ldsy = h->req.ldsy;
    c->req.nt = h->req.nt;
    c->req.xwin = 0;
    c->req.slab = 0;
    c->opt.mode = h->opt.mode;
    c->opt.xcd_remap = 1;
}

int convert_child(SlabBuild &b)
{
    csr5hip_handle h = b.h;
    SlabStructure &sl = h->slab;
    const Geometry &g = h->g;
    hipStream_t s = h->stream;
    const bool hot = b.choice.verdict == SLAB_TABLE;
    csr5hip_handle c = sl.child ? sl.child : new csr5hip_handle_s();
    sl.child = c;
    c->is_child = true;
    c->g.m = (int)b.m2;
    c->g.n = g.n;
    c->value_type = h->value_type;
    c->stream = s;
    inherit_child(c, h);
    c->hot_enabled = hot;
    c->d.col_lo = hot ? (const uint16_t *)sl[B_COL_LO].ptr : nullptr;
    c->d.col_hi = hot ? (const uint8_t *)sl[B_COL_HI].ptr : nullptr;
    c->d.slab_off = (const int32_t *)sl[B_SLAB_OFF].ptr;
    c->d.slab_shift = h->req.slab_shift;
    c->d.slab_bits = b.choice.bits;
    c->d.xperm = hot ? sl[B_XPERM].ptr : nullptr;
    c->d.cold_base = hot ? (const int32_t *)sl[B_COLD_BASE].ptr : nullptr;
    c->d.cold_cols = hot ? (const int32_t *)sl[B_COLD_COLS].ptr : nullptr;
    c->d.cold_total = hot ? sl.cold_total : 0;
    sl.xperm_valid = false;
    c->d.hot_cols = (const int32_t *)sl[B_HOT_COLS].ptr;
    c->d.hot_count = (const int32_t *)sl[B_HOT_COUNT].ptr;
    c->d.hot_tile0 = (const int32_t *)sl[B_HOT_TILE0].ptr;
    c->d.hot_slabs = b.choice.S;
    c->d.hot_capacity = b.plan.hot_capacity;
    c->d.range_lead = sl[B_LEAD].ptr;
    c->d.range_head = (uint32_t *)sl[B_RANGE_HEAD].ptr;
    int rc = csr5hip_input_csr(c, g.nnz, (int32_t *)sl[B_ROW_PTR2].ptr, (int32_t *)sl[B_COL2].ptr, sl[B_VAL2].ptr);
    c->sigma_request = hot ? b.plan.hot_sigma : g.sigma;
    if (rc == CSR5HIP_SUCCESS)
        rc = csr5hip_as_csr5(c);
    if (rc == CSR5HIP_SUCCESS && hot) {
        hipError_t e = launch_range_heads(c->g, c->d, s);
        if (e == hipSuccess)
            e = hipStreamSynchronize(s);
        if (e != hipSuccess)
            rc = fail_hip(e, "k_range_heads");
    }
    return rc;
}

int narrow_values(SlabBuild &b)
{
    csr5hip_handle h = b.h, c = h->slab.child;
    h->slab.values_narrowed = false;
    c->d.val32 = nullptr;
    if (!(b.choice.verdict == SLAB_TABLE && h->req.narrow && h->value_type == CSR5HIP_F64 && h->g.nnz > 0))
        return CSR5HIP_SUCCESS;
    bool narrow = false, copying = false;
    const hipError_t e = narrow_child_values(h, c, true, &narrow, &copying);
    if (e != hipSuccess)
        return fail_hip(e, "narrow values");
    if (narrow) {
        c->d.val32 = (const float *)h->slab[B_VAL32].ptr;
        h->slab.values_narrowed = true;
    }
    return CSR5HIP_SUCCESS;
}

int build_slabs_impl(csr5hip_handle h)
{
    SlabStructure &sl = h->slab;
    sl.deactivate();
    sl.t_slab = 0;
    const double t0 = now_ms();
    SlabBuild b{};
    b.h = h;
    int rc = plan_slabs(h, &b.plan);
    if (rc != CSR5HIP_SUCCESS)
        return rc;
    if (!b.plan.S) {
        sl.release();
        return CSR5HIP_SUCCESS;
    }
    rc = reserve_temporaries(b);
    if (rc != CSR5HIP_SUCCESS)
        return rc;
    struct TmpGuard {
        Buffer &b;
        size_t keep;
        ~TmpGuard()
        {
            if (b.cap > keep)
                b.release();
        }
    } tmp_guard{sl[B_TMP], b.tmp_keep};
    if (b.plan.hot) {
        rc = select_hot_columns(b);
        if (rc != CSR5HIP_SUCCESS)
            return rc;
    }
    b.choice = slab_after_sample(b.plan, sl.hot_cover_pct);
    if (b.choice.verdict == SLAB_NONE) {
        sl.t_slab = now_ms() - t0;
        return CSR5HIP_SUCCESS;
    }
    rc = partition_segments(b);
    if (rc == CSR5HIP_SUCCESS && b.choice.verdict == SLAB_TABLE)
        rc = deal_and_pack(b);
    if (rc != CSR5HIP_SUCCESS)
        return rc;
    HIP_TRY(hipStreamSynchronize(h->stream));
    rc = convert_child(b);
    if (rc == CSR5HIP_SUCCESS)
        rc = narrow_values(b);
    if (rc != CSR5HIP_SUCCESS)
        return rc;
    csr5hip_handle c = sl.child;
    if (c->hot_enabled) {
        const hipError_t e = prepare_spmv_hot(c->g, c->d, c->value_type, c->opt);
        if (e != hipSuccess)
            return fail_hip(e, "LDS limit of the range kernel");
    }
    sl.S = b.choice.S;
    sl.m2 = (int)b.m2;
    sl.t_slab = now_ms() - t0;
    return CSR5HIP_SUCCESS;
}

}

namespace csr5 {

int build_slabs(csr5hip_handle h)
{
    h->slab.fallback = false;
    const int rc = build_slabs_impl(h);
    if (rc == CSR5HIP_SUCCESS)
        return h->slab.S > 0 || h->is_child ? rc : prepare_plain(h);
    const std::string why = last_error();
    (void)hipGetLastError();
    h->slab.release();
    h->slab.fallback = true;
    h->drop_graphs();
    set_last_error("column slabs not built, plain tile kernel in use: " + why);
    if (h->req.slab >= 2)
        return rc;
    return prepare_plain(h);
}

hipError_t narrow_child_values(csr5hip_handle h, csr5hip_handle c, bool sync_copy, bool *narrow, bool *copying)
{
    *narrow = *copying = false;
    hipStream_t s = h->stream;
    const size_t nnz = (size_t)h->g.nnz;
    unsigned *flag = c->d.counters + 5;
    unsigned inexact = 1;
    hipError_t e = launch_fp32_exact((const double *)c->d.val, nnz, flag, s);
    if (e == hipSuccess)
        e = hipMemcpyAsync(&inexact, flag, sizeof(inexact), hipMemcpyDeviceToHost, s);
    if (e == hipSuccess)
        e = hipStreamSynchronize(s);
    if (e != hipSuccess || inexact)
        return e;
    *copying = true;
    e = h->slab[B_VAL32].reserve(nnz * sizeof(float));
    if (e == hipSuccess)
        e = launch_narrow((const double *)c->d.val, nnz, (float *)h->slab[B_VAL32].ptr, c->g.tile_elems, c->g.p - 1, s);
    if (e == hipSuccess && sync_copy)
        e = hipStreamSynchronize(s);
    *narrow = e == hipSuccess;
    return e;
}

}
```

Before: 491.4.

## Replace 32-bit slab row keys with byte flags and row bytes in slab build

The slab partition now writes a one-byte segment-start flag and a one-byte low row index per nonzero instead of a 32-bit key. Runs that continue across tiles are resolved by a separate kernel that compares per-tile first and last rows. Segment counting and emitting read 16 flags per thread, and the base table is recomputed from row_ptr and the column slab counts instead of searching the keys. This targets memory traffic in the preprocessing stage, not the SpMV kernel itself, so the measured GFLOPS may not change.

```diff
diff --git a/benchmark_spmv_using_csr5_amd/csrc/csr5_internal.h b/benchmark_spmv_using_csr5_amd/csrc/csr5_internal.h
--- a/benchmark_spmv_using_csr5_amd/csrc/csr5_internal.h
+++ b/benchmark_spmv_using_csr5_amd/csrc/csr5_internal.h
@@ -104,11 +104,12 @@
 hipError_t slab_select_tmp_bytes(int nnz, size_t *bytes);
 hipError_t slab_partition(const Geometry &g, const DeviceArrays &d, int value_type, int S, int bits, int shift,
                           uint32_t *hist, void *scan_tmp, size_t scan_tmp_bytes, int32_t *col2, void *val2,
-                          uint32_t *key2, hipStream_t s);
-hipError_t slab_count_segments(int nnz, const uint32_t *key2, void *tmp, unsigned int *d_count, hipStream_t s);
-hipError_t slab_segments(int nnz, const uint32_t *key2, const void *tmp, int32_t *row_ptr2, unsigned char *rowidx, hipStream_t s);
+                          uint8_t *flag, uint8_t *rowb, int32_t *run_first, int32_t *run_last, hipStream_t s);
+hipError_t slab_count_segments(int nnz, const uint8_t *flag, void *tmp, unsigned int *d_count, hipStream_t s);
+hipError_t slab_segments(int nnz, const uint8_t *flag, const uint8_t *rowb, const void *tmp, int32_t *row_ptr2, unsigned char *rowidx,
+                         hipStream_t s);
 size_t slab_base_words(int m, int S);
-hipError_t slab_tables(int m, int m2, int nnz, int S, int p, const int32_t *row_ptr, int32_t *row_ptr2, const uint32_t *key2,
+hipError_t slab_tables(const Geometry &g, const DeviceArrays &d, int m2, int S, int bits, int shift, int32_t *row_ptr2,
                        const uint32_t *chunk_start, uint32_t *base, uint32_t *nonempty, hipStream_t s);
 hipError_t slab_hot_select(int n, int nnz, int S, int bits, int shift, int capacity, int min_count, int sample_stride,
                            const int32_t *col, uint32_t *cnt, void *hotmap, uint32_t *chist, uint32_t *thr,
@@ -118,7 +119,7 @@
 size_t slab_cold_words(int n, int S, int bits, int shift);
 hipError_t slab_cold_sort_tmp_bytes(size_t total, int slab_bits, size_t *bytes);
 hipError_t slab_hot_pack(int n, int nnz, int T, int p, int S, int bits, int shift, const int32_t *slab_off, const void *hotmap,
-                         const uint32_t *cnt, const uint32_t *key2, int32_t *col2, uint16_t *col_lo, uint8_t *col_hi, uint8_t *ref, uint32_t *rank_of,
+                         const uint32_t *cnt, const uint8_t *flag, int32_t *col2, uint16_t *col_lo, uint8_t *col_hi, uint8_t *ref, uint32_t *rank_of,
                          uint32_t *keys, uint32_t *keys_sorted, uint32_t *src_sorted, void *sort_tmp, size_t sort_tmp_bytes,
                          int32_t *cold_base, int32_t *cold_cols, hipStream_t s);
 size_t slab_local_columns(int n, int bits, int shift);
diff --git a/benchmark_spmv_using_csr5_amd/csrc/csr5_slab.hip b/benchmark_spmv_using_csr5_amd/csrc/csr5_slab.hip
--- a/benchmark_spmv_using_csr5_amd/csrc/csr5_slab.hip
+++ b/benchmark_spmv_using_csr5_amd/csrc/csr5_slab.hip
@@ -9,7 +9,7 @@
 
 constexpr int SLAB_BLOCK = 256;
 constexpr int SLAB_MAX = 64;
-constexpr uint32_t SLAB_KEY_FIRST = 0x80000000u;
+constexpr int COMBINE_ROWS = 256;
 
 __host__ __device__ inline size_t slab_hot_groups(int n, int shift, int bits) { return (slab_local_count(n, shift, bits) + 127) / 128; }
 __device__ __forceinline__ bool hot_lookup(const uint4 w, uint32_t bit, uint32_t &below)
@@ -101,7 +101,8 @@
 k_slab_scatter(Geometry g, const int32_t *__restrict__ row_ptr, const uint32_t *__restrict__ tile_ptr,
                const int32_t *__restrict__ col, const VT *__restrict__ val, int S, int bits, int shift,
                const uint32_t *__restrict__ chunk_start, int32_t *__restrict__ col2, VT *__restrict__ val2,
-               uint32_t *__restrict__ key2)
+               uint8_t *__restrict__ flag, uint8_t *__restrict__ rowb, int32_t *__restrict__ run_first,
+               int32_t *__restrict__ run_last)
 {
     extern __shared__ __attribute__((aligned(16))) char smem[];
     const int T = g.tile_elems;
@@ -113,7 +114,7 @@
     unsigned char *srank = skey + T;
     constexpr int ROWCAP = 1024;
     __shared__ int32_t srow[ROWCAP];
-    __shared__ uint32_t slab_first[SLAB_MAX], gstart[SLAB_MAX], lstart[SLAB_MAX + 1];
+    __shared__ uint32_t gstart[SLAB_MAX], lstart[SLAB_MAX + 1];
 
     const int t = blockIdx.x;
     const int tid = threadIdx.x, lane = tid & (OMEGA - 1), wave = tid >> 6;
@@ -127,10 +128,8 @@
         sval[c] = val[base + q];
         skey[c] = (unsigned char)slab_of((uint32_t)ci, shift, bits);
     }
-    if (tid < S) {
-        slab_first[tid] = chunk_start[(size_t)tid * g.p];
+    if (tid < S)
         gstart[tid] = chunk_start[(size_t)tid * g.p + t];
-    }
     const int rs = (int)(tile_ptr[t] & ROW_MASK);
     const int re = (int)(tile_ptr[t + 1] & ROW_MASK);
     const bool rows_in_lds = re - rs <= ROWCAP;
@@ -175,45 +174,85 @@
         inv[lstart[k] + off[(c >> 6) * S + k] + srank[c]] = (uint16_t)c;
     }
     __syncthreads();
-    for (int o = tid; o < E; o += SLAB_BLOCK) {
-        const int c = inv[o];
-        const int k = skey[c];
-        const size_t dst = (size_t)gstart[k] + ((uint32_t)o - lstart[k]);
-        const int j = (int)(base + c);
-        const int row = rs + (rows_in_lds ? upper_bound_i32(srow, j, re - rs) : upper_bound_i32(row_ptr + rs + 1, j, re - rs));
-        col2[dst] = scol[c];
-        val2[dst] = sval[c];
-        key2[dst] = (uint32_t)row | (dst == slab_first[k] ? SLAB_KEY_FIRST : 0u);
-    }
-}
-
-__device__ __forceinline__ bool key_starts(uint32_t a, uint32_t before)
-{
-    return (a & SLAB_KEY_FIRST) != 0 || ((a ^ before) & ~SLAB_KEY_FIRST) != 0;
-}
-__device__ __forceinline__ unsigned segment_starts4(const uint32_t *__restrict__ key, long long j, long long hi, uint32_t k[4])
+    auto row_of = [&](int o) -> int {
+        const int j = (int)(base + inv[o]);
+        return rs + (rows_in_lds ? upper_bound_i32(srow, j, re - rs) : upper_bound_i32(row_ptr + rs + 1, j, re - rs));
+    };
+    const int per = (E + SLAB_BLOCK - 1) / SLAB_BLOCK * OMEGA;
+    const int o_begin = wave * per, o_end = o_begin + per < E ? o_begin + per : E;
+    int carry = o_begin > 0 && o_begin < E ? row_of(o_begin - 1) : -1;
+    for (int o0 = o_begin; o0 < o_end; o0 += OMEGA) {
+        const int o = o0 + lane;
+        const bool valid = o < o_end;
+        const int row = valid ? row_of(o) : -1;
+        int before = __shfl_up(row, 1, OMEGA);
+        before = lane == 0 ? carry : before;
+        carry = __shfl(row, OMEGA - 1, OMEGA);
+        if (valid) {
+            const int c = inv[o];
+            const int k = skey[c];
+            const size_t dst = (size_t)gstart[k] + ((uint32_t)o - lstart[k]);
+            const bool run_starts = (uint32_t)o == lstart[k];
+            col2[dst] = scol[c];
+            val2[dst] = sval[c];
+            flag[dst] = run_starts || before != row ? 1 : 0;
+            rowb[dst] = (uint8_t)(row & (COMBINE_ROWS - 1));
+            if (run_starts)
+                run_first[(size_t)t * S + k] = row;
+            if ((uint32_t)o + 1 == lstart[k + 1])
+                run_last[(size_t)t * S + k] = row;
+        }
+    }
+}
+
+__global__ void __launch_bounds__(SLAB_BLOCK)
+k_slab_resolve_runs(int S, int p, int nnz, const uint32_t *__restrict__ chunk_start, const int32_t *__restrict__ run_first,
+                    const int32_t *__restrict__ run_last, uint8_t *__restrict__ flag)
+{
+    const long long e = (long long)blockIdx.x * SLAB_BLOCK + threadIdx.x;
+    if (e >= (long long)S * p)
+        return;
+    const int t = (int)(e / S), k = (int)(e % S);
+    const uint32_t *cs = chunk_start + (size_t)k * p;
+    const uint32_t start = cs[t], end = t + 1 < p || k + 1 < S ? cs[t + 1] : (uint32_t)nnz;
+    if (start == end || start == cs[0])
+        return;
+    int before = t - 1;
+    if (cs[before] == start) {
+        int lo = 0, hi = t;
+        while (lo < hi) {
+            const int mid = (lo + hi) >> 1;
+            if (cs[mid] < start)
+                lo = mid + 1;
+            else
+                hi = mid;
+        }
+        before = lo - 1;
+    }
+    if (run_last[(size_t)before * S + k] == run_first[e])
+        flag[start] = 0;
+}
+
+__device__ __forceinline__ unsigned flag_nibble(uint32_t v) { return (v & 1u) | ((v >> 7) & 2u) | ((v >> 14) & 4u) | ((v >> 21) & 8u); }
+__device__ __forceinline__ unsigned flag_starts4(const uint8_t *__restrict__ flag, long long j, long long hi)
 {
     if (j >= hi)
         return 0u;
-    const uint32_t before = j > 0 ? key[j - 1] : 0u;
-    if (j + 4 <= hi) {
-        const uint4 v = *reinterpret_cast<const uint4 *>(key + j);
-        k[0] = v.x, k[1] = v.y, k[2] = v.z, k[3] = v.w;
-    } else {
-        for (int i = 0; i < 4; i++)
-            k[i] = j + i < hi ? key[j + i] : 0u;
-    }
-    unsigned f = j == 0 || key_starts(k[0], before) ? 1u : 0u;
-#pragma unroll
-    for (int i = 1; i < 4; i++)
-        f |= (j + i < hi && key_starts(k[i], k[i - 1]) ? 1u : 0u) << i;
-    return f;
-}
-
-constexpr int COMBINE_ROWS = 256;
+    const unsigned f = flag_nibble(*reinterpret_cast<const uint32_t *>(flag + j));
+    return j + 4 > hi ? f & ((1u << (int)(hi - j)) - 1u) : f;
+}
+__device__ __forceinline__ unsigned flag_starts16(const uint8_t *__restrict__ flag, long long j, long long hi)
+{
+    if (j >= hi)
+        return 0u;
+    const uint4 v = *reinterpret_cast<const uint4 *>(flag + j);
+    const unsigned f = flag_nibble(v.x) | (flag_nibble(v.y) << 4) | (flag_nibble(v.z) << 8) | (flag_nibble(v.w) << 12);
+    return j + 16 > hi ? f & ((1u << (int)(hi - j)) - 1u) : f;
+}
 
 constexpr int SEG_BLOCKS = 2048;
-constexpr int SEG_STEP = SLAB_BLOCK * 4;
+constexpr int SEG_STEP = SLAB_BLOCK * 16;
+constexpr int SEG_AHEAD = 4;
 __host__ __device__ inline long long seg_chunk(int nnz, int blocks)
 {
     long long c = ((long long)nnz + blocks - 1) / blocks;
@@ -221,20 +260,25 @@
 }
 static int seg_blocks(int nnz)
 {
-    long long b = ((long long)nnz + 4095) / 4096;
+    long long b = ((long long)nnz + SEG_STEP - 1) / SEG_STEP;
     return (int)(b < 1 ? 1 : (b > SEG_BLOCKS ? SEG_BLOCKS : b));
 }
 
 __global__ void __launch_bounds__(SLAB_BLOCK)
-k_slab_count_segments(int nnz, const uint32_t *__restrict__ key, unsigned int *__restrict__ block_count)
+k_slab_count_segments(int nnz, const uint8_t *__restrict__ flag, unsigned int *__restrict__ block_count)
 {
     __shared__ unsigned part[SLAB_BLOCK / OMEGA];
     const long long chunk = seg_chunk(nnz, gridDim.x);
     const long long lo = (long long)blockIdx.x * chunk, hi = lo + chunk < nnz ? lo + chunk : nnz;
     unsigned local = 0;
-    for (long long j = lo + (long long)threadIdx.x * 4; j < hi; j += SEG_STEP) {
-        uint32_t k[4];
-        local += (unsigned)__popc(segment_starts4(key, j, hi, k));
+    for (long long j = lo + (long long)threadIdx.x * 16; j < hi; j += (long long)SEG_AHEAD * SEG_STEP) {
+        unsigned f[SEG_AHEAD];
+#pragma unroll
+        for (int u = 0; u < SEG_AHEAD; u++)
+            f[u] = flag_starts16(flag, j + (long long)u * SEG_STEP, hi);
+#pragma unroll
+        for (int u = 0; u < SEG_AHEAD; u++)
+            local += (unsigned)__popc(f[u]);
     }
 #pragma unroll
     for (int d = 32; d >= 1; d >>= 1)
@@ -287,8 +331,9 @@
 }
 
 __global__ void __launch_bounds__(SLAB_BLOCK)
-k_slab_emit_segments(int nnz, const uint32_t *__restrict__ key, const unsigned int *__restrict__ block_offset,
-                     int32_t *__restrict__ row_ptr2, unsigned char *__restrict__ rowidx)
+k_slab_emit_segments(int nnz, const uint8_t *__restrict__ flag, const uint8_t *__restrict__ rowb,
+                     const unsigned int *__restrict__ block_offset, int32_t *__restrict__ row_ptr2,
+                     unsigned char *__restrict__ rowidx)
 {
     __shared__ unsigned wave_count[SLAB_BLOCK / OMEGA];
     const long long chunk = seg_chunk(nnz, gridDim.x);
@@ -296,9 +341,11 @@
     const int lane = threadIdx.x & (OMEGA - 1), w = threadIdx.x / OMEGA;
     unsigned out = block_offset[blockIdx.x];
     for (long long j0 = lo; j0 < hi; j0 += SEG_STEP) {
-        const long long j = j0 + (long long)threadIdx.x * 4;
-        uint32_t k4[4];
-        const unsigned f = segment_starts4(key, j, hi, k4);
+        const long long j = j0 + (long long)threadIdx.x * 16;
+        unsigned f = flag_starts16(flag, j, hi);
+        uint4 rb = make_uint4(0, 0, 0, 0);
+        if (j < hi)
+            rb = *reinterpret_cast<const uint4 *>(rowb + j);
         const unsigned own = (unsigned)__popc(f);
         unsigned incl = own;
 #pragma unroll
@@ -316,51 +363,58 @@
             all += wave_count[k];
         }
         unsigned at = out + before + incl - own;
-#pragma unroll
-        for (int i = 0; i < 4; i++)
-            if (f & (1u << i)) {
-                row_ptr2[at] = (int32_t)(j + i);
-                rowidx[at++] = (unsigned char)(k4[i] & (COMBINE_ROWS - 1));
-            }
+        const unsigned long long rb_lo = (unsigned long long)rb.x | ((unsigned long long)rb.y << 32);
+        const unsigned long long rb_hi = (unsigned long long)rb.z | ((unsigned long long)rb.w << 32);
+        while (f) {
+            const int i = __builtin_ctz(f);
+            f &= f - 1u;
+            row_ptr2[at] = (int32_t)(j + i);
+            rowidx[at++] = (unsigned char)((i < 8 ? rb_lo : rb_hi) >> (8 * (i & 7)));
+        }
         out += all;
         __syncthreads();
     }
 }
 
+constexpr int BASE_WAVES = SLAB_BLOCK / OMEGA;
 __global__ void __launch_bounds__(SLAB_BLOCK)
-k_slab_base(int m2, int nnz, int S, int nblk, const int32_t *__restrict__ row_ptr2, const uint32_t *__restrict__ key,
-            const uint32_t *__restrict__ chunk_start, int p, uint32_t *__restrict__ base, int32_t *__restrict__ row_ptr2_end)
-{
-    __shared__ int slab_seg[SLAB_MAX + 1];
+k_slab_base(Geometry g, int m2, int S, int bits, int shift, int nblk, const int32_t *__restrict__ row_ptr,
+            const uint32_t *__restrict__ tile_ptr, const int32_t *__restrict__ col, const int32_t *__restrict__ row_ptr2,
+            const uint32_t *__restrict__ chunk_start, uint32_t *__restrict__ base, int32_t *__restrict__ row_ptr2_end)
+{
+    __shared__ uint32_t cnt[BASE_WAVES][SLAB_MAX];
     if (blockIdx.x == 0 && threadIdx.x == 0)
-        *row_ptr2_end = nnz;
-    if ((int)threadIdx.x <= S) {
-        const uint32_t first = (int)threadIdx.x < S ? chunk_start[(size_t)threadIdx.x * p] : (uint32_t)nnz;
-        int lo = 0, hi = m2;
-        while (lo < hi) {
-            const int mid = (int)(((unsigned)lo + (unsigned)hi) >> 1);
-            if ((uint32_t)row_ptr2[mid] < first)
-                lo = mid + 1;
-            else
-                hi = mid;
-        }
-        slab_seg[threadIdx.x] = lo;
-    }
-    __syncthreads();
-    const long long e = (long long)blockIdx.x * SLAB_BLOCK + threadIdx.x;
-    if (e >= (long long)(nblk + 1) * S)
+        *row_ptr2_end = g.nnz;
+    const int lane = threadIdx.x & (OMEGA - 1), w = threadIdx.x >> 6;
+    const int b = blockIdx.x * BASE_WAVES + w;
+    if (b > nblk)
         return;
-    const int b = (int)(e / S), k = (int)(e % S);
-    const uint32_t want = (uint32_t)b * COMBINE_ROWS;
-    int lo = slab_seg[k], hi = slab_seg[k + 1];
+    const long long r = (long long)b * COMBINE_ROWS;
+    const int e = row_ptr[r < g.m ? r : g.m];
+    const bool inside = e < g.nnz;
+    const int t = inside ? e / g.tile_elems : 0, c0 = inside ? e - t * g.tile_elems : 0;
+    cnt[w][lane] = 0;
+    if (c0 > 0) {
+        const bool tr = tile_is_transposed(g, tile_ptr, t);
+        const size_t tile0 = (size_t)t * g.tile_elems;
+        for (int c = lane; c < c0; c += OMEGA) {
+            const int q = tr ? (c % g.sigma) * OMEGA + c / g.sigma : c;
+            atomicAdd(&cnt[w][slab_of((uint32_t)col[tile0 + q], shift, bits)], 1u);
+        }
+    }
+    if (lane >= S)
+        return;
+    const uint32_t pos = inside ? chunk_start[(size_t)lane * g.p + t] + cnt[w][lane]
+                                : (lane + 1 < S ? chunk_start[(size_t)(lane + 1) * g.p] : (uint32_t)g.nnz);
+    int lo = 0, hi = m2;
     while (lo < hi) {
         const int mid = (int)(((unsigned)lo + (unsigned)hi) >> 1);
-        if ((key[row_ptr2[mid]] & ~SLAB_KEY_FIRST) < want)
+        if ((uint32_t)row_ptr2[mid] < pos)
             lo = mid + 1;
         else
             hi = mid;
     }
-    base[e] = (uint32_t)lo;
+    base[(size_t)b * S + lane] = (uint32_t)lo;
 }
 
 __global__ void __launch_bounds__(SLAB_BLOCK)
@@ -794,7 +848,7 @@
 k_hot_encode(int nnz, int T, int p, int S, int bits, int shift, const int32_t *__restrict__ slab_off,
              const uint4 *__restrict__ hotbits, const uint16_t *__restrict__ hotpre, size_t G, int32_t *__restrict__ col2,
              uint16_t *__restrict__ col_lo, uint8_t *__restrict__ col_hi, uint8_t *__restrict__ ref,
-             const uint32_t *__restrict__ rank_of, size_t L, const uint32_t *__restrict__ key)
+             const uint32_t *__restrict__ rank_of, size_t L, const uint8_t *__restrict__ flag)
 {
     extern __shared__ __attribute__((aligned(16))) char smem[];
     uint4 *lbits = reinterpret_cast<uint4 *>(smem);
@@ -866,8 +920,7 @@
                     v[u].z = encode(v[u].z, pos + 2);
                     v[u].w = encode(v[u].w, pos + 3);
                     if (MODE == ENC_PACK) {
-                        uint32_t k4[4];
-                        const unsigned st = segment_starts4(key, pos, (long long)nnz, k4);
+                        const unsigned st = flag_starts4(flag, pos, (long long)nnz);
                         const uint32_t a = (uint32_t)v[u].x | ((st & 1u) << 22), b = (uint32_t)v[u].y | (((st >> 1) & 1u) << 22),
                                        c = (uint32_t)v[u].z | (((st >> 2) & 1u) << 22), d = (uint32_t)v[u].w | (((st >> 3) & 1u) << 22);
                         lo4[q] = make_uint2((a & 0xFFFFu) | (b << 16), (c & 0xFFFFu) | (d << 16));
@@ -948,7 +1001,7 @@
 
 hipError_t slab_partition(const Geometry &g, const DeviceArrays &d, int value_type, int S, int bits, int shift,
                           uint32_t *hist, void *scan_tmp, size_t scan_tmp_bytes, int32_t *col2, void *val2,
-                          uint32_t *key2, hipStream_t s)
+                          uint8_t *flag, uint8_t *rowb, int32_t *run_first, int32_t *run_last, hipStream_t s)
 {
     const size_t hist_lds = (size_t)(SLAB_BLOCK / OMEGA) * S * HIST_PAD * 4;
     hipError_t e = hipFuncSetAttribute(reinterpret_cast<const void *>(k_slab_hist), hipFuncAttributeMaxDynamicSharedMemorySize,
@@ -967,10 +1020,13 @@
     const size_t lds = slab_scatter_lds(g, S, vs);
     if (value_type == CSR5HIP_F64)
         hipLaunchKernelGGL(k_slab_scatter<double>, dim3(g.p), dim3(SLAB_BLOCK), lds, s, g, d.row_ptr, d.tile_ptr, d.col,
-                           (const double *)d.val, S, bits, shift, hist, col2, (double *)val2, key2);
+                           (const double *)d.val, S, bits, shift, hist, col2, (double *)val2, flag, rowb, run_first, run_last);
     else
         hipLaunchKernelGGL(k_slab_scatter<float>, dim3(g.p), dim3(SLAB_BLOCK), lds, s, g, d.row_ptr, d.tile_ptr, d.col,
-                           (const float *)d.val, S, bits, shift, hist, col2, (float *)val2, key2);
+                           (const float *)d.val, S, bits, shift, hist, col2, (float *)val2, flag, rowb, run_first, run_last);
+    const long long runs = (long long)S * g.p;
+    hipLaunchKernelGGL(k_slab_resolve_runs, dim3((unsigned)((runs + SLAB_BLOCK - 1) / SLAB_BLOCK)), dim3(SLAB_BLOCK), 0, s, S, g.p, g.nnz, hist,
+                       run_first, run_last, flag);
     return hipGetLastError();
 }
 
@@ -986,29 +1042,30 @@
     return hipSuccess;
 }
 
-hipError_t slab_count_segments(int nnz, const uint32_t *key2, void *tmp, unsigned int *d_count, hipStream_t s)
+hipError_t slab_count_segments(int nnz, const uint8_t *flag, void *tmp, unsigned int *d_count, hipStream_t s)
 {
     const int blocks = seg_blocks(nnz);
-    hipLaunchKernelGGL(k_slab_count_segments, dim3(blocks), dim3(SLAB_BLOCK), 0, s, nnz, key2, (unsigned int *)tmp);
+    hipLaunchKernelGGL(k_slab_count_segments, dim3(blocks), dim3(SLAB_BLOCK), 0, s, nnz, flag, (unsigned int *)tmp);
     hipLaunchKernelGGL(k_slab_scan_counts, dim3(1), dim3(1024), 0, s, blocks, (unsigned int *)tmp, d_count);
     return hipGetLastError();
 }
 
-hipError_t slab_segments(int nnz, const uint32_t *key2, const void *tmp, int32_t *row_ptr2, unsigned char *rowidx, hipStream_t s)
-{
-    hipLaunchKernelGGL(k_slab_emit_segments, dim3(seg_blocks(nnz)), dim3(SLAB_BLOCK), 0, s, nnz, key2,
+hipError_t slab_segments(int nnz, const uint8_t *flag, const uint8_t *rowb, const void *tmp, int32_t *row_ptr2, unsigned char *rowidx,
+                         hipStream_t s)
+{
+    hipLaunchKernelGGL(k_slab_emit_segments, dim3(seg_blocks(nnz)), dim3(SLAB_BLOCK), 0, s, nnz, flag, rowb,
                        (const unsigned int *)tmp, row_ptr2, rowidx);
     return hipGetLastError();
 }
 
 size_t slab_base_words(int m, int S) { return ((size_t)(m + COMBINE_ROWS - 1) / COMBINE_ROWS + 2) * (size_t)S; }
-hipError_t slab_tables(int m, int m2, int nnz, int S, int p, const int32_t *row_ptr, int32_t *row_ptr2, const uint32_t *key2,
+hipError_t slab_tables(const Geometry &g, const DeviceArrays &d, int m2, int S, int bits, int shift, int32_t *row_ptr2,
                        const uint32_t *chunk_start, uint32_t *base, uint32_t *nonempty, hipStream_t s)
 {
-    const int nblk = (m + COMBINE_ROWS - 1) / COMBINE_ROWS;
-    const long long entries = (long long)(nblk + 1) * S;
-    hipLaunchKernelGGL(k_slab_base, dim3((unsigned)((entries + SLAB_BLOCK - 1) / SLAB_BLOCK)), dim3(SLAB_BLOCK), 0, s, m2, nnz, S,
-                       nblk, row_ptr2, key2, chunk_start, p, base, row_ptr2 + m2);
+    const int m = g.m, nblk = (m + COMBINE_ROWS - 1) / COMBINE_ROWS;
+    const int32_t *row_ptr = d.row_ptr;
+    hipLaunchKernelGGL(k_slab_base, dim3((unsigned)(nblk + 1 + BASE_WAVES - 1) / BASE_WAVES), dim3(SLAB_BLOCK), 0, s, g, m2, S, bits, shift,
+                       nblk, row_ptr, d.tile_ptr, d.col, row_ptr2, chunk_start, base, row_ptr2 + m2);
     hipLaunchKernelGGL(k_slab_nonempty, dim3((m + 32 + SLAB_BLOCK - 1) / SLAB_BLOCK), dim3(SLAB_BLOCK), 0, s, m, row_ptr, nonempty);
     return hipGetLastError();
 }
@@ -1098,7 +1155,7 @@
 
 static hipError_t hot_encode_pass(int mode, int n, int nnz, int T, int p, int S, int bits, int shift, const int32_t *slab_off,
                                   const void *hotmap, int32_t *col2, uint16_t *col_lo, uint8_t *col_hi, uint8_t *ref,
-                                  const uint32_t *rank_of, const uint32_t *key, hipStream_t s)
+                                  const uint32_t *rank_of, const uint8_t *flag, hipStream_t s)
 {
     const size_t G = slab_hot_groups(n, shift, bits);
     const size_t L = slab_local_count(n, shift, bits);
@@ -1115,7 +1172,7 @@
                 return e;
         }
         hipLaunchKernelGGL(kern, grid, block, in_lds ? lds : 0, s, nnz, T, p, S, bits, shift, slab_off, hotbits, hotpre, G, col2,
-                           col_lo, col_hi, ref, rank_of, L, key);
+                           col_lo, col_hi, ref, rank_of, L, flag);
         return hipGetLastError();
     };
     if (mode == ENC_MARK)
@@ -1132,7 +1189,7 @@
 }
 
 hipError_t slab_hot_pack(int n, int nnz, int T, int p, int S, int bits, int shift, const int32_t *slab_off, const void *hotmap,
-                         const uint32_t *cnt, const uint32_t *key2, int32_t *col2, uint16_t *col_lo, uint8_t *col_hi, uint8_t *ref, uint32_t *rank_of,
+                         const uint32_t *cnt, const uint8_t *flag, int32_t *col2, uint16_t *col_lo, uint8_t *col_hi, uint8_t *ref, uint32_t *rank_of,
                          uint32_t *keys, uint32_t *keys_sorted, uint32_t *src_sorted, void *sort_tmp, size_t sort_tmp_bytes,
                          int32_t *cold_base, int32_t *cold_cols, hipStream_t s)
 {
@@ -1151,7 +1208,7 @@
     e = hipGetLastError();
     if (e != hipSuccess)
         return e;
-    return hot_encode_pass(ENC_PACK, n, nnz, T, p, S, bits, shift, slab_off, hotmap, col2, col_lo, col_hi, nullptr, rank_of, key2, s);
+    return hot_encode_pass(ENC_PACK, n, nnz, T, p, S, bits, shift, slab_off, hotmap, col2, col_lo, col_hi, nullptr, rank_of, flag, s);
 }
 
 size_t slab_local_columns(int n, int bits, int shift) { return slab_local_count(n, shift, bits); }
diff --git a/benchmark_spmv_using_csr5_amd/csrc/csr5_slab_build.hip b/benchmark_spmv_using_csr5_amd/csrc/csr5_slab_build.hip
--- a/benchmark_spmv_using_csr5_amd/csrc/csr5_slab_build.hip
+++ b/benchmark_spmv_using_csr5_amd/csrc/csr5_slab_build.hip
@@ -62,7 +62,12 @@
     size_t tmp_keep;
     SlabChoice choice;
     unsigned int m2;
+    size_t runs_off, runs_bytes;
     void *tmp(SlabRegion r) const { return (char *)h->slab[B_TMP].ptr + arena.off[r]; }
+    uint8_t *flags() const { return (uint8_t *)tmp(T_KEY); }
+    uint8_t *row_bytes() const { return flags() + (((size_t)h->g.nnz + 31) & ~(size_t)15); }
+    int32_t *run_first() const { return (int32_t *)((char *)h->slab[B_TMP].ptr + runs_off); }
+    int32_t *run_last() const { return (int32_t *)((char *)h->slab[B_TMP].ptr + runs_off + runs_bytes / 2); }
     void *covered() const { return (char *)h->slab[B_TMP].ptr + arena.covered(); }
 };
 
@@ -107,9 +112,13 @@
     }
     sz.base_words = slab_base_words(g.m, pl.S_alloc);
     b.arena = slab_arena(pl, sz);
-    if (h->req.slab_mem_mib > 0 && !slab_memory_fits(slab_memory_need(pl, sz, b.arena.total), h->req.slab_mem_mib))
+    b.runs_off = b.arena.total;
+    b.runs_bytes = 2 * (((size_t)pl.S_alloc * g.p * 4 + 255) & ~(size_t)255);
+    if (2 * ((size_t)g.nnz + 31) > b.arena.bytes[T_KEY])
+        return fail_hip(hipErrorInvalidValue, "column slabs: the flag and row bytes do not fit their region");
+    if (h->req.slab_mem_mib > 0 && !slab_memory_fits(slab_memory_need(pl, sz, b.arena.total + b.runs_bytes), h->req.slab_mem_mib))
         return fail_hip(hipErrorOutOfMemory, "column slabs: CSR5HIP_OPT_SLAB_MEMORY_MIB");
-    HIP_TRY(h->slab[B_TMP].reserve(b.arena.total));
+    HIP_TRY(h->slab[B_TMP].reserve(b.arena.total + b.runs_bytes));
     return CSR5HIP_SUCCESS;
 }
 
@@ -149,22 +158,22 @@
     const Geometry &g = h->g;
     hipStream_t s = h->stream;
     const int S = b.choice.S;
-    const uint32_t *key = (const uint32_t *)b.tmp(T_KEY), *hist = (const uint32_t *)b.tmp(T_HIST);
+    const uint32_t *hist = (const uint32_t *)b.tmp(T_HIST);
     HIP_TRY(sl[B_COL2].reserve((size_t)g.nnz * 4));
     HIP_TRY(sl[B_VAL2].reserve((size_t)g.nnz * h->vsize()));
     HIP_TRY(slab_partition(g, h->d, h->value_type, S, b.choice.bits, h->req.slab_shift, (uint32_t *)b.tmp(T_HIST), b.tmp(T_SCAN), b.sz.scan,
-                           (int32_t *)sl[B_COL2].ptr, sl[B_VAL2].ptr, (uint32_t *)b.tmp(T_KEY), s));
-    HIP_TRY(slab_count_segments(g.nnz, key, b.tmp(T_SEL), (unsigned int *)b.tmp(T_COUNT), s));
+                           (int32_t *)sl[B_COL2].ptr, sl[B_VAL2].ptr, b.flags(), b.row_bytes(), b.run_first(), b.run_last(), s));
+    HIP_TRY(slab_count_segments(g.nnz, b.flags(), b.tmp(T_SEL), (unsigned int *)b.tmp(T_COUNT), s));
     unsigned int m2 = 0;
     HIP_TRY(hipMemcpyAsync(&m2, b.tmp(T_COUNT), 4, hipMemcpyDeviceToHost, s));
     HIP_TRY(hipStreamSynchronize(s));
     b.m2 = m2;
     HIP_TRY(sl[B_ROW_PTR2].reserve(((size_t)m2 + 1) * 4));
     HIP_TRY(sl[B_ROWIDX].reserve((size_t)m2 + 1));
-    HIP_TRY(slab_segments(g.nnz, key, b.tmp(T_SEL), (int32_t *)sl[B_ROW_PTR2].ptr, (unsigned char *)sl[B_ROWIDX].ptr, s));
+    HIP_TRY(slab_segments(g.nnz, b.flags(), b.row_bytes(), b.tmp(T_SEL), (int32_t *)sl[B_ROW_PTR2].ptr, (unsigned char *)sl[B_ROWIDX].ptr, s));
     HIP_TRY(sl[B_BASE].reserve(slab_base_words(g.m, S) * 4));
     HIP_TRY(sl[B_NONEMPTY].reserve(((size_t)g.m / 32 + 16) * 4));
-    HIP_TRY(slab_tables(g.m, (int)m2, g.nnz, S, g.p, h->d.row_ptr, (int32_t *)sl[B_ROW_PTR2].ptr, key, hist, (uint32_t *)sl[B_BASE].ptr,
+    HIP_TRY(slab_tables(g, h->d, (int)m2, S, b.choice.bits, h->req.slab_shift, (int32_t *)sl[B_ROW_PTR2].ptr, hist, (uint32_t *)sl[B_BASE].ptr,
                         (uint32_t *)sl[B_NONEMPTY].ptr, s));
     HIP_TRY(sl[B_P].reserve(((size_t)m2 + 1) * h->vsize()));
     HIP_TRY(hipMemsetAsync(sl[B_P].ptr, 0, ((size_t)m2 + 1) * h->vsize(), s));
@@ -195,7 +204,7 @@
     HIP_TRY(sl[B_XPERM].reserve(((size_t)S * pl.hot_capacity + cold_cap + (size_t)pl.hot_T + 1) * h->vsize()));
     HIP_TRY(hipMemsetAsync(b.tmp(T_REF), 0, b.sz.cold_words, s));
     HIP_TRY(slab_hot_pack(g.n, g.nnz, pl.hot_T, pl.hot_p, S, b.choice.bits, h->req.slab_shift, (const int32_t *)sl[B_SLAB_OFF].ptr,
-                          b.tmp(T_HOTMAP), (const uint32_t *)b.tmp(T_CNT), (const uint32_t *)b.tmp(T_KEY), (int32_t *)sl[B_COL2].ptr,
+                          b.tmp(T_HOTMAP), (const uint32_t *)b.tmp(T_CNT), b.flags(), (int32_t *)sl[B_COL2].ptr,
                           (uint16_t *)sl[B_COL_LO].ptr, (uint8_t *)sl[B_COL_HI].ptr, (uint8_t *)b.tmp(T_REF), (uint32_t *)b.tmp(T_RANK),
                           (uint32_t *)b.tmp(T_KEYS), (uint32_t *)b.tmp(T_KEYS2), (uint32_t *)b.tmp(T_SRC), b.tmp(T_SORT), b.sz.cold_sort,
                           (int32_t *)sl[B_COLD_BASE].ptr, (int32_t *)sl[B_COLD_COLS].ptr, s));
```

Result: no change. 490.8 (-0.1%).
